# fdrmrc/fictitious_domain_AL_preconditioners

Hardware: AMD Instinct MI355X
Metric: FGMRES iterations/sec to 1e-8 residual, 3D Stokes-immersed (AL-preconditioned) (higher is better)
Workload: dtype f64

## Files before the change

### fictitious_domain_al_preconditioners_amd/_abi.py

```python
import ctypes as C

ALFD_MAX_BLOCKS = 3

OK, E_INVALID, E_HIP, E_NO_CONVERGENCE_OUTER, E_NO_CONVERGENCE_INNER, E_BREAKDOWN, E_NOT_SETUP, \
    E_COMM, E_UNSUPPORTED = range(9)
A, BT, B, CT, C_, M, MP, A2, KIMM = range(9)
NSLOTS = 9
SLOT_BY_NAME = {"A": A, "Bt": BT, "B": B, "Ct": CT, "C": C_, "M": M, "Mp": MP, "A2": A2, "K": KIMM}
INVW, MP_LUMPED_INV = 0, 1
NDIAGS = 2
AL2, AL_STOKES, AL_STOKES_DIAG, AL_ELL_IDEAL, AL_ELL_MODIFIED, RATIONAL = range(6)
CTRL_ABS, CTRL_REDUCTION, CTRL_FIXED_ITERS = range(3)
PREC_IDENTITY, PREC_JACOBI, PREC_CHEBYSHEV, PREC_MULTILEVEL = range(4)
INNER_OP_AUG, INNER_OP_A22, INNER_OP_AUG2 = range(3)
SPECTRUM_CCT = 0
ORTH_MGS, ORTH_CGS, ORTH_CGS2 = range(3)
OUTER_FGMRES, OUTER_MINRES = range(2)
FGMRES_DEALII_96, FGMRES_DEALII_95 = range(2)
W_DIAGONAL, W_MASS_INV_SQUARED, W_MASS_INV = range(3)
INNER_THROW, INNER_ACCEPT = range(2)
T_SPMV_A, T_SPMV_OTHER, T_DOT, T_VEC = range(4)
T_NCLASSES = 4
SC_PRODUCTS_A, SC_PRODUCTS_C, SC_LEVEL_A_UPLOADS, SC_TRANSFER_UPLOADS, SC_PATCH_BUILDS, SC_POWER_ITERATIONS = range(6)
SC_NCOUNTS = 6
SETUP_COUNT_NAMES = ("products_a", "products_c", "level_a_uploads", "transfer_uploads", "patch_builds",
                     "power_iterations")
UNIQUE_ID_BYTES = 128


class Control(C.Structure):
    _fields_ = [("kind", C.c_int32), ("max_steps", C.c_int32), ("tol", C.c_double), ("reduce", C.c_double)]

    def __init__(self, kind=CTRL_ABS, max_steps=100, tol=1e-10, reduce=0.0):
        super().__init__(kind, max_steps, tol, reduce)


class Config(C.Structure):
    _fields_ = [
        ("variant", C.c_int32), ("restart", C.c_int32), ("orthogonalization", C.c_int32),
        ("grad_div_in_A", C.c_int32),
        ("gamma", C.c_double), ("gamma_grad_div", C.c_double), ("gamma2", C.c_double),
        ("outer", Control), ("inner", Control), ("mp_inner", Control),
        ("inner_prec", C.c_int32), ("cheb_degree", C.c_int32), ("cheb_power_its", C.c_int32),
        ("on_inner_failure", C.c_int32),
        ("cheb_eig_ratio", C.c_double), ("cheb_safety", C.c_double),
        ("log_level", C.c_int32), ("outer_solver", C.c_int32),
        ("rho_bound", C.c_double), ("rational", Control),
        ("ml_smooth_degree", C.c_int32), ("ml_coarse_degree", C.c_int32),
        ("ml_smooth_ratio", C.c_double), ("ml_coarse_ratio", C.c_double),
        ("aug_assembled", C.c_int32), ("w_inverse", C.c_int32),
        ("mass", Control),
        ("fgmres_flavour", C.c_int32), ("ml_smooth_degree_coarse", C.c_int32),
        ("ml_patch_degree", C.c_int32), ("ml_coarse_direct", C.c_int32), ("ml_patch_ratio", C.c_double),
    ]


class Result(C.Structure):
    _fields_ = [
        ("status", C.c_int32), ("outer_iterations", C.c_int32),
        ("initial_residual", C.c_double), ("last_residual", C.c_double),
        ("inner_iterations", C.c_int64), ("mp_iterations", C.c_int64),
        ("inner_failures", C.c_int32), ("precond_applications", C.c_int32),
        ("solve_seconds", C.c_double), ("lambda_max", C.c_double),
        ("rational_iterations", C.c_int64), ("mass_iterations", C.c_int64),
    ]

    def as_dict(self):
        return {k: getattr(self, k) for k, _ in self._fields_}


class Spectrum(C.Structure):
    _fields_ = [
        ("converged", C.c_int32), ("steps", C.c_int32),
        ("initial_residual", C.c_double), ("last_residual", C.c_double),
        ("lambda_min", C.c_double), ("lambda_max", C.c_double), ("condition", C.c_double),
    ]

    def as_dict(self):
        return {k: getattr(self, k) for k, _ in self._fields_}


class MatrixInfo(C.Structure):
    _fields_ = [
        ("lanes", C.c_int32), ("windowed", C.c_int32), ("value_indexed", C.c_int32), ("batch_major", C.c_int32),
        ("nnz", C.c_int64), ("window_blocks", C.c_int64), ("window_fallback_blocks", C.c_int64),
        ("value_indexed_blocks", C.c_int64), ("value_indexed_nnz", C.c_int64),
        ("dictionary_entries", C.c_int64), ("value_wide_nnz", C.c_int64),
        ("algorithmic_bytes", C.c_double), ("streamed_bytes", C.c_double),
        ("shared_nnz", C.c_int64), ("batch_major_blocks", C.c_int64), ("batch_major_wide", C.c_int64),
        ("batch_major_interior_blocks", C.c_int64),
    ]


class BatchMajorShape(C.Structure):
    _fields_ = [
        ("batch_major", C.c_int32), ("lanes", C.c_int32),
        ("nrows", C.c_int64), ("nnz", C.c_int64), ("shared_nnz", C.c_int64),
        ("rows", C.c_int64), ("waves", C.c_int64), ("small", C.c_int64),
        ("blocks", C.c_int64), ("batches", C.c_int64), ("lds_bytes", C.c_int64), ("compute_units", C.c_int64),
    ]

    def as_dict(self):
        plain = ("batch_major", "lanes", "nrows", "nnz", "shared_nnz")
        return {(k if k in plain else "batch_major_" + k): getattr(self, k) for k, _ in self._fields_}


OPERATOR_LEVEL, OPERATOR_PATCH_SS, OPERATOR_PATCH_S = 0, 1, 2


class WindowPlanInfo(C.Structure):
    _fields_ = [
        ("windowed", C.c_int32), ("value_indexed", C.c_int32), ("row_block", C.c_int32), ("max_window", C.c_int32),
        ("blocks", C.c_int64), ("fallback_blocks", C.c_int64), ("segments", C.c_int64),
        ("value_indexed_blocks", C.c_int64), ("value_indexed_nnz", C.c_int64), ("value_wide_nnz", C.c_int64),
        ("dictionary_entries", C.c_int64), ("batches", C.c_int64), ("decode_mismatches", C.c_int64),
    ]


class StreamPlanInfo(C.Structure):
    _fields_ = [
        ("ok", C.c_int32), ("max_window", C.c_int32), ("max_rows", C.c_int32), ("max_batches", C.c_int32),
        ("blocks", C.c_int64), ("batches", C.c_int64), ("segments", C.c_int64), ("dictionary_entries", C.c_int64),
        ("stream_bytes", C.c_int64), ("decode_mismatches", C.c_int64), ("rows_covered", C.c_int64),
        ("shared_nnz", C.c_int64),
    ]


def default_config(variant=AL_STOKES) -> Config:
    c = Config()
    c.variant = variant
    c.restart = 50 if variant in (AL_ELL_IDEAL, AL_ELL_MODIFIED) else 30
    c.orthogonalization = ORTH_CGS2
    c.grad_div_in_A = 1
    c.gamma, c.gamma_grad_div, c.gamma2 = 10.0, 10.0, 1e-2
    c.outer = Control(CTRL_REDUCTION, 1000, 1e-8, 1e-12)
    c.inner = Control(CTRL_ABS, 100, 1e-2, 0.0)
    c.mp_inner = Control(CTRL_ABS, 100, 1e-6, 0.0)
    c.inner_prec = PREC_CHEBYSHEV
    c.cheb_degree = 4
    c.cheb_power_its = 20
    c.on_inner_failure = INNER_THROW
    c.cheb_eig_ratio = 30.0
    c.cheb_safety = 1.2
    c.log_level = 0
    c.outer_solver = OUTER_MINRES if variant == RATIONAL else OUTER_FGMRES
    c.rho_bound = 0.0
    c.rational = Control(CTRL_ABS, 2000, 1e-14, 0.0)
    c.ml_smooth_degree, c.ml_coarse_degree = 3, 40
    c.ml_smooth_ratio, c.ml_coarse_ratio = 4.0, 400.0
    c.w_inverse = W_DIAGONAL
    c.mass = Control(CTRL_REDUCTION, 1000, 1e-30, 1e-14)
    c.ml_patch_degree, c.ml_coarse_direct, c.ml_patch_ratio = 0, 0, 30.0
    return c


def bench_multilevel_settings(cfg: Config, geometric: bool = True) -> Config:
    cfg.inner_prec = PREC_MULTILEVEL
    cfg.inner.max_steps = 100
    cfg.ml_coarse_degree = 10
    if geometric:
        cfg.ml_smooth_degree, cfg.ml_smooth_degree_coarse, cfg.ml_smooth_ratio = 3, 5, 40.0
        cfg.ml_patch_degree, cfg.ml_patch_ratio, cfg.ml_coarse_direct = 15, 200.0, 1024
    else:
        cfg.ml_smooth_degree, cfg.ml_smooth_degree_coarse, cfg.ml_smooth_ratio = 4, 0, 256.0
        cfg.ml_patch_degree, cfg.ml_coarse_direct = 0, 0
    return cfg


BENCH_MIN_COARSE = 1024
```

### fictitious_domain_al_preconditioners_amd/csrc/alfd.hip

```cpp

#include <hip/hip_runtime.h>
#include <rccl/rccl.h>

#include <algorithm>
#include <atomic>
#include <chrono>
#include <cmath>
#include <cstdio>
#include <cstdlib>
#include <cstring>
#include <memory>
#include <climits>
#include <condition_variable>
#include <functional>
#include <limits>
#include <mutex>
#include <string>
#include <thread>
#include <unordered_set>
#include <vector>

#include "alfd/alfd.h"
#include "kernels.hpp"
#include "kernels_vs.hpp"

namespace alfd {


#define HIPC(call)                                                                          \
  do {                                                                                      \
    hipError_t e__ = (call);                                                                \
    if (e__ != hipSuccess) {                                                                \
      ctx->err = std::string(#call) + ": " + hipGetErrorString(e__) + " (" + __FILE__ + ":" + \
                 std::to_string(__LINE__) + ")";                                            \
      return ALFD_E_HIP;                                                                    \
    }                                                                                       \
  } while (0)
#define RC(call)                  \
  do {                            \
    int rc__ = (call);            \
    if (rc__ != ALFD_OK) return rc__; \
  } while (0)

static inline int64_t pad_chunk(int64_t n) { return (n + kChunk - 1) / kChunk * kChunk; }

struct DevCsr {
  bool present = false;
  int64_t nrows = 0, ncols = 0, nnz = 0;
  int64_t n_list = 0;
  bool sparse = false;
  bool rep = false;
  bool derived = false;
  int L = 64;
  int32_t n_local_cols = 0;
  int64_t *rp = nullptr;
  int32_t *col = nullptr;
  double *val = nullptr;
  int32_t *rows = nullptr;
  std::vector<int64_t> send_off, recv_off;
  std::vector<int32_t> halo_globals;
  int32_t *send_idx = nullptr;
  double *send_buf = nullptr, *halo = nullptr;
  int64_t n_halo = 0;
  std::vector<void *> owned;
  bool win = false;
  bool win_deferred = false, win_user = true;
  int tag = 0;
  int32_t win_RB = 0, win_maxW = 0;
  int64_t win_nblocks = 0, win_fallback_blocks = 0, win_nseg = 0;
  uint16_t *lcol = nullptr;
  bool vi = false;
  uint8_t *vidx = nullptr;
  int32_t *blk_dict_off = nullptr, *blk_dict_n = nullptr;
  double *dict = nullptr;
  int64_t vi_blocks = 0, vi_nnz = 0, vi_dict_total = 0, vi_wide_nnz = 0;
  uint16_t *vidw = nullptr;
  uint64_t *vib_tab = nullptr;
  int32_t *vib_cnt = nullptr;
  int32_t vib_stride = 0;
  int32_t *blk_seg_begin = nullptr, *blk_W = nullptr, *seg_col = nullptr, *seg_off = nullptr;
  struct Vs {
    bool on = false, bricks = false;
    int64_t nb = 0, nseg = 0, stream_bytes = 0, nbatch = 0, dict_total = 0, shared_nnz = 0;
    int32_t stride = 0, maxW = 0;
    int32_t L = 64, tab_u64 = 16;
    int32_t wide = 0;
    int32_t RB = 0, NW = 4;
    bool small = false;
    uint8_t *stream = nullptr;
    int64_t *sb = nullptr;
    uint64_t *tab = nullptr;
    int32_t *cnt = nullptr, *seg_begin = nullptr, *blkW = nullptr, *seg_col = nullptr,
            *seg_off = nullptr, *doff = nullptr, *dn = nullptr;
    int32_t *hdrb = nullptr, *segx = nullptr;
    int32_t seg_stride = 0;
    int64_t nb_interior = 0;
    double *dict = nullptr;
  } vs;
  double streamed_bytes(bool use_vi, bool use_vs = false) const {
    const double vec = (double)(n_list + 1) * 8.0 + (double)n_list * 8.0 + (double)(sparse ? n_list : ncols) * 8.0;
    if (vs.on && use_vs && use_vi)
      return (double)vs.stream_bytes + 8.0 * vs.tab_u64 * (double)vs.nbatch + 28.0 * (double)vs.nb +
             8.0 * (double)vs.nseg + 8.0 * (double)vs.dict_total + 8.0 * (double)nrows +
             8.0 * (double)(sparse ? n_list : ncols);
    if (!win) return (double)nnz * 12.0 + vec;
    const double meta = (double)win_nblocks * 8.0 + (double)win_nseg * 8.0;
    if (!(vi && use_vi)) return (double)nnz * 10.0 + vec + meta;
    return (double)(vi_nnz - vi_wide_nnz) * 3.0 + (double)vi_wide_nnz * 4.0 + (double)(nnz - vi_nnz) * 10.0 + vec + meta + (double)vi_dict_total * 8.0 +
           (double)win_nblocks * (8.0 + (vib_tab ? 32.0 * vib_stride + 4.0 : 0.0));
  }
  double algorithmic_bytes() const {
    return (double)nnz * 12.0 + (double)(n_list + 1) * 8.0 + (double)n_list * 8.0 +
           (double)(sparse ? n_list : ncols) * 8.0;
  }
};

struct HostCsr {
  int64_t nrows = 0, ncols = 0;
  std::vector<int64_t> rp;
  std::vector<int32_t> col;
  std::vector<double> val;
  int64_t nnz() const { return rp.empty() ? 0 : rp.back(); }
};

constexpr int kScratchSlot = ALFD_NSLOTS;

struct LevelStore {
  DevCsr A, C, Ct;
  DevCsr P, R;
  int64_t n = 0, npad = 0;
  double *dinv = nullptr, *r = nullptr, *z = nullptr, *t = nullptr, *cd = nullptr, *cres = nullptr, *ctmp = nullptr;
};

struct MlLevel {
  LevelStore loc, rep;
  double lmax = 0;
  uint8_t *tail_mask = nullptr;
  bool P_global_cols = false;
  std::vector<int64_t> offs;
  int64_t maxpiece = 0;
  double *send = nullptr, *stage = nullptr;
};

enum State { ITERATE = 0, SUCCESS = 1, FAILURE = 2 };
struct Control {
  alfd_control c;
  double initial = 0, reduced_tol = 0, last_value = 0;
  int last_step = 0;
  State check(int step, double v) {
    last_step = step;
    last_value = v;
    if (step == 0) {
      initial = v;
      reduced_tol = v * c.reduce;
    }
    if (c.kind == ALFD_CTRL_REDUCTION && v < reduced_tol) return SUCCESS;
    if (c.kind == ALFD_CTRL_FIXED_ITERS && step >= c.max_steps) return SUCCESS;
    if (v <= c.tol) return SUCCESS;
    if (step >= c.max_steps || std::isnan(v)) return FAILURE;
    return ITERATE;
  }
};

struct TimedLaunch {
  int cls;
  hipEvent_t a, b;
};

}

using namespace alfd;

struct alfd_ctx {
  int device = 0;
  hipStream_t stream = nullptr;
  hipStream_t xstream = nullptr;
  hipEvent_t ev_x = nullptr, ev_halo = nullptr;
  hipEvent_t ev_in = nullptr;
  int overlap_halo = -1;
  std::string err;
  int rank = 0, nranks = 1;
  ncclComm_t nccl = nullptr;
// ... 56 lines not shown
    void clear_input() {
      for (int l = 0; l < ALFD_MAX_LEVELS; ++l) agg[l].clear(), wgt[l].clear(), P[l] = HostCsr(), ncoarse[l] = 0;
      built_partitioned = false;
    }
  } hier[2];
  struct Patch {
    bool on = false;
    int64_t m = 0, mpad = 0;
    DevCsr Ass, As, Ats, Cs, Cts;
    int32_t *S = nullptr;
    double *dinv = nullptr, *rS = nullptr, *zS = nullptr, *uS = nullptr, *eS = nullptr, *cd = nullptr,
           *cres = nullptr, *ctmp = nullptr, *rr = nullptr;
    double lmax = 0;
    uint8_t *tail_mask = nullptr;
    bool rep = false;
    int64_t m_loc = 0, piece = 1, lam_piece = 1;
    std::vector<int64_t> soff;
    DevCsr Cts_loc, Ctg;
    double *send = nullptr, *stage = nullptr, *lam_send = nullptr, *lam_stage = nullptr, *loc = nullptr;
  } patch;
  struct StrengthGraph {
    bool have = false, on_device = false;
    int64_t n_nodes = 0, node0 = 0;
    std::vector<int64_t> gp;
    std::vector<int32_t> gc, fixed;
    std::vector<double> gw, d;
  } sg;
  int ml_rep_level = -1;
  bool dots_replicated = false;
  int64_t ml_rep_threshold = 300000;
  int ml_fuse = 2;
  int ml_tail_rows = 0;
  int ml_gpu_galerkin = 1;
  double *g_w = nullptr, *g_tlam = nullptr;
  std::vector<int64_t> ml_coff[ALFD_MAX_LEVELS];
  const int64_t *up_col_offsets = nullptr;
  bool up_local_only = false;
  DevCsr rat_mat;
  double *rt_r = nullptr, *rt_z = nullptr, *rt_p = nullptr, *rt_Ap = nullptr, *rt_x = nullptr;
  double *rt_dinv = nullptr, *rt_partial = nullptr, *rt_scb = nullptr, *rt_coef = nullptr;
  double *rt_scb_host = nullptr;
  int64_t rational_its = 0;
  int64_t wmax = 0;
  std::vector<void *> ws_allocs;
  double *w_r = nullptr, *w_z = nullptr, *w_p = nullptr, *w_Ap = nullptr;
  double *c_d = nullptr, *c_res = nullptr, *c_tmp = nullptr;
  double *t_lam = nullptr;
  double *q_tmp = nullptr, *rhs_tmp = nullptr;
  double *V = nullptr, *Z = nullptr, *xb = nullptr, *bb = nullptr, *io = nullptr;
  double *st_in = nullptr, *st_out = nullptr;
  double lambda_max = 0, lambda_min = 0;
  int64_t inner_its = 0, mp_its = 0;
  int64_t inner_its_op[3] = {0, 0, 0};
  int inner_failures = 0, precond_applications = 0;
  std::vector<double> history;
  int timing = 0;
  std::vector<TimedLaunch> timed;
  double t_ms[ALFD_T_NCLASSES] = {0, 0, 0, 0};
  int64_t t_launches[ALFD_T_NCLASSES] = {0, 0, 0, 0};
  double t_bytes[ALFD_T_NCLASSES] = {0, 0, 0, 0};
  double t_fbytes[ALFD_T_NCLASSES] = {0, 0, 0, 0};
  double setup_s[ALFD_SETUP_NPHASES] = {0, 0, 0, 0, 0, 0, 0, 0};
  bool upload_since_setup = false;
  uint64_t gen[ALFD_NSLOTS + 1] = {}, gen_setup[ALFD_NSLOTS + 1] = {};
  uint64_t dgen[ALFD_NDIAGS] = {}, dgen_setup[ALFD_NDIAGS] = {};
  alfd_config cfg_setup;
  const char *needs_full = nullptr;
  bool coupling_ready = false;
  int64_t setup_counts[ALFD_SC_NCOUNTS] = {};
  std::vector<void *> cp_allocs[2];
  std::vector<void *> allocs;
  int spmv_stream_R = 2, spmv_stream_U = 8, spmv_nt = 0, spmv_grid_mult = 8;
  int spmv_group_R = 4, spmv_group_U = 4;
  bool vi_off = false;
  int vi_rows_R = 4, vi_rows_J = 2;
  int vi_xcd = 0;
  int vi_levels = 1;
  int vi_batched = 1;
  int win_RB_vi = 96;
  int win_vi = 1;
  int win_short_scale = 2;
  int vs_enable = 1, vs_NW = 4, vs_RB = 96, vs_xcd = 0, vs_share = 1, vs_wide = 1;
  int vs_small = 1;
  int vs_cus = 0;
  int vs_force_RB = 0, vs_force_NW = 0;
  int vs_lds_base_ok = -1;
  std::vector<int64_t> rb_ptr[ALFD_NSLOTS + 1];
  std::vector<int32_t> rb_rows[ALFD_NSLOTS + 1];
  int win_short_min_blocks = 256;
  int win_min_blocks = 256;
  int win_enable = 1, win_RB = 96, win_maxW = 4096, win_gap = 8, win_xcd = 0;
  int64_t ntot() const { return off[nblocks]; }
};

struct alfd_local_group {
  int n = 0;
  std::mutex mu;
  std::condition_variable cv;
  int arrived = 0;
  long generation = 0;
  std::vector<const void *> buf;
  std::vector<const int64_t *> off;
  void barrier() {
    std::unique_lock<std::mutex> lk(mu);
    const long g = generation;
    if (++arrived == n) {
      arrived = 0;
      ++generation;
      cv.notify_all();
    } else {
      cv.wait(lk, [&] { return generation != g; });
    }
  }
};

namespace alfd {

static int comm_allgather(alfd_ctx *ctx, const void *send, void *recv, size_t bytes) {
  if (ctx->local) {
    alfd_local_group *g = ctx->local;
    HIPC(hipStreamSynchronize(ctx->stream));
    g->buf[ctx->rank] = send;
    g->barrier();
    for (int p = 0; p < g->n; ++p)
      HIPC(hipMemcpyAsync((char *)recv + (size_t)p * bytes, g->buf[p], bytes, hipMemcpyDeviceToDevice,
                          ctx->stream));
    HIPC(hipStreamSynchronize(ctx->stream));
    g->barrier();
    return ALFD_OK;
  }
  if (ctx->host_allgather) {
    ctx->host_send.resize(bytes);
    ctx->host_recv.resize(bytes * (size_t)ctx->nranks);
    HIPC(hipMemcpyAsync(ctx->host_send.data(), send, bytes, hipMemcpyDeviceToHost, ctx->stream));
    HIPC(hipStreamSynchronize(ctx->stream));
    if (ctx->host_allgather(ctx->host_user, ctx->host_send.data(), ctx->host_recv.data(), bytes) != 0)
      return ctx->err = "host all-gather callback failed", ALFD_E_COMM;
    HIPC(hipMemcpyAsync(recv, ctx->host_recv.data(), ctx->host_recv.size(), hipMemcpyHostToDevice, ctx->stream));
    HIPC(hipStreamSynchronize(ctx->stream));
    return ALFD_OK;
  }
  if (ncclAllGather(send, recv, bytes, ncclChar, ctx->nccl, ctx->stream) != ncclSuccess)
    return ctx->err = "ncclAllGather failed", ALFD_E_COMM;
  return ALFD_OK;
}

static int comm_alltoallv(alfd_ctx *ctx, const void *sendbuf, const int64_t *send_off, void *recvbuf,
                          const int64_t *recv_off, size_t es, hipStream_t st = nullptr) {
  if (!st) st = ctx->stream;
  if (ctx->local) {
    alfd_local_group *g = ctx->local;
    HIPC(hipStreamSynchronize(st));
    g->buf[ctx->rank] = sendbuf;
    g->off[ctx->rank] = send_off;
    g->barrier();
    for (int p = 0; p < g->n; ++p) {
      const int64_t nr = recv_off[p + 1] - recv_off[p];
      if (nr > 0)
        HIPC(hipMemcpyAsync((char *)recvbuf + (size_t)recv_off[p] * es,
                            (const char *)g->buf[p] + (size_t)g->off[p][ctx->rank] * es, (size_t)nr * es,
                            hipMemcpyDeviceToDevice, st));
    }
    HIPC(hipStreamSynchronize(st));
    g->barrier();
    return ALFD_OK;
  }
// ... 56 lines not shown
  for (void *q : m.owned) hipFree(q);
  m = DevCsr();
}

static void spectrum_release(alfd_ctx *ctx) {
  csr_free(ctx->spec.own_Cs);
  csr_free(ctx->spec.own_Cts);
  for (void *q : ctx->spec.owned) hipFree(q);
  ctx->spec = alfd_ctx::Spectrum();
}

static inline int grid_for_rows(int64_t nrows, int L) {
  const int64_t groups = (nrows + (kBlock / L) - 1) / (kBlock / L);
  return (int)std::max<int64_t>(1, std::min<int64_t>(groups, 256 * 8));
}

struct Timer {
  alfd_ctx *ctx;
  int cls;
  hipEvent_t a = nullptr, b = nullptr;
  bool on;
  Timer(alfd_ctx *c, int cl, double bytes, double fbytes = -1.0) : ctx(c), cls(cl) {
    on = ctx->timing >= 2 || (ctx->timing == 1 && cl == ALFD_T_SPMV_A);
    if (on) {
      hipEventCreate(&a);
      hipEventCreate(&b);
      hipEventRecord(a, ctx->stream);
      ctx->t_bytes[cls] += bytes;
      ctx->t_fbytes[cls] += fbytes < 0.0 ? bytes : fbytes;
      ctx->t_launches[cls]++;
    }
  }
  ~Timer() {
    if (on) {
      hipEventRecord(b, ctx->stream);
      ctx->timed.push_back({cls, a, b});
    }
  }
};

struct PhaseClock {
  alfd_ctx *ctx;
  int phase;
  std::chrono::steady_clock::time_point t0 = std::chrono::steady_clock::now();
  PhaseClock(alfd_ctx *c, int ph) : ctx(c), phase(ph) {}
  ~PhaseClock() {
    hipStreamSynchronize(ctx->stream);
    ctx->setup_s[phase] += std::chrono::duration<double>(std::chrono::steady_clock::now() - t0).count();
  }
};

static void flush_timers(alfd_ctx *ctx) {
  for (auto &t : ctx->timed) {
    hipEventSynchronize(t.b);
    float ms = 0;
    hipEventElapsedTime(&ms, t.a, t.b);
    ctx->t_ms[t.cls] += ms;
    hipEventDestroy(t.a);
    hipEventDestroy(t.b);
  }
  ctx->timed.clear();
}

template <int L>
static void launch_spmv_L(alfd_ctx *ctx, const DevCsr &m, const double *x, double *y, int epi, double alpha,
                          const double *d, double *y2) {
  const int grid = grid_for_rows(m.n_list, L);
  const double *xh = m.halo;
#define ALFD_SPMV(EPI, SP)                                                                          \
  hipLaunchKernelGGL((spmv_kernel<L, EPI, SP>), dim3(grid), dim3(kBlock), 0, ctx->stream, m.n_list, \
                     m.rp, m.col, m.val, m.rows, x, xh, m.n_local_cols, y, alpha, d, y2)
  if (m.sparse) {
    if (epi == 0) ALFD_SPMV(0, true);
    else if (epi == 1) ALFD_SPMV(1, true);
    else if (epi == 2) ALFD_SPMV(2, true);
    else ALFD_SPMV(3, true);
  } else {
    if (epi == 0) ALFD_SPMV(0, false);
    else if (epi == 1) ALFD_SPMV(1, false);
    else if (epi == 2) ALFD_SPMV(2, false);
    else ALFD_SPMV(3, false);
  }
#undef ALFD_SPMV
}

template <int R, int U, bool NT>
static void launch_stream(alfd_ctx *ctx, const DevCsr &m, const double *x, double *y, int epi, double alpha,
                          const double *d, double *y2) {
  const int64_t nbatches = (m.nrows + R - 1) / R;
  const int grid = (int)std::max<int64_t>(1, std::min<int64_t>((nbatches + 3) / 4, 256 * ctx->spmv_grid_mult));
#define ALFD_STREAM(EPI)                                                                              \
  hipLaunchKernelGGL((spmv_stream_kernel<R, U, EPI, NT>), dim3(grid), dim3(kBlock), 0, ctx->stream,   \
                     m.nrows, m.rp, m.col, m.val, x, m.halo, m.n_local_cols, y, alpha, d, y2, NoPair())
  if (epi == 0) ALFD_STREAM(0);
  else if (epi == 1) ALFD_STREAM(1);
  else if (epi == 2) ALFD_STREAM(2);
  else ALFD_STREAM(3);
#undef ALFD_STREAM
}

template <bool NT>
static bool launch_stream_RU(alfd_ctx *ctx, const DevCsr &m, const double *x, double *y, int epi,
                             double alpha, const double *d, double *y2) {
  const int R = ctx->spmv_stream_R, U = ctx->spmv_stream_U;
#define ALFD_RU(RR, UU) \
  if (R == RR && U == UU) return launch_stream<RR, UU, NT>(ctx, m, x, y, epi, alpha, d, y2), true
  ALFD_RU(2, 2); ALFD_RU(2, 4); ALFD_RU(4, 2); ALFD_RU(4, 4); ALFD_RU(4, 8); ALFD_RU(8, 4); ALFD_RU(8, 8);
  ALFD_RU(1, 4); ALFD_RU(2, 8); ALFD_RU(8, 2);
#undef ALFD_RU
  return false;
}

template <int R, int U>
static void launch_window(alfd_ctx *ctx, const DevCsr &m, const double *x, double *y, int epi, double alpha,
                          const double *d, double *y2) {
  const size_t lds = (size_t)(m.win_maxW + (m.vi && !ctx->vi_off ? kDictMaxEntries : 0)) * sizeof(double);
#define ALFD_WIN(EPI, TAG)                                                                              \
  hipLaunchKernelGGL((spmv_window_kernel<R, U, EPI, TAG>), dim3((unsigned)m.win_nblocks), dim3(kBlock), \
                     lds, ctx->stream, m.nrows, m.win_RB, m.rp, m.col, m.lcol, m.val, m.blk_seg_begin,   \
                     m.blk_W, m.seg_col, m.seg_off, x, m.halo, m.n_local_cols, y, alpha, d, y2, ctx->win_xcd)
  const bool vi = m.vi && !ctx->vi_off;
  if (vi && ctx->vi_batched && m.vib_tab) {
#define ALFD_VIB(EPI, TAG)                                                                                    \
  hipLaunchKernelGGL((spmv_window_vib_kernel<EPI, TAG>), dim3((unsigned)m.win_nblocks), dim3(kBlock), lds,   \
                     ctx->stream, m.nrows, m.win_RB, m.rp, m.col, m.lcol, m.val, m.blk_seg_begin, m.blk_W,    \
                     m.seg_col, m.seg_off, x, m.halo, m.n_local_cols, y, alpha, d, y2, m.vidx, m.vidw,        \
                     m.blk_dict_off, m.blk_dict_n, m.dict, m.win_maxW, m.vib_tab, m.vib_cnt, m.vib_stride,    \
                     ctx->vi_xcd)
    if (m.tag == 0) {
      if (epi == 0) ALFD_VIB(0, 0);
      else if (epi == 1) ALFD_VIB(1, 0);
      else if (epi == 2) ALFD_VIB(2, 0);
      else ALFD_VIB(3, 0);
    } else {
      if (epi == 0) ALFD_VIB(0, 1);
      else if (epi == 1) ALFD_VIB(1, 1);
      else if (epi == 2) ALFD_VIB(2, 1);
      else ALFD_VIB(3, 1);
    }
#undef ALFD_VIB
    return;
  }
  if (vi && ctx->vi_rows_R > 0) {
    const int RR = ctx->vi_rows_R, JJ = ctx->vi_rows_J;
#define ALFD_VI(RV, JV, EPI)                                                                                  \
  hipLaunchKernelGGL((spmv_window_vi_kernel<RV, JV, EPI>), dim3((unsigned)m.win_nblocks), dim3(kBlock), lds,  \
                     ctx->stream, m.nrows, m.win_RB, m.rp, m.col, m.lcol, m.val, m.blk_seg_begin, m.blk_W,     \
                     m.seg_col, m.seg_off, x, m.halo, m.n_local_cols, y, alpha, d, y2, m.vidx, m.vidw, \
                     m.blk_dict_off, m.blk_dict_n, m.dict, m.win_maxW)
#define ALFD_VI_E(RV, JV)              \
  if (RR == RV && JJ == JV) {          \
    if (epi == 0) ALFD_VI(RV, JV, 0);  \
    else if (epi == 1) ALFD_VI(RV, JV, 1); \
    else if (epi == 2) ALFD_VI(RV, JV, 2); \
    else ALFD_VI(RV, JV, 3);           \
    return;                            \
  }
    ALFD_VI_E(4, 3) ALFD_VI_E(2, 4) ALFD_VI_E(4, 4)
    if (epi == 0) ALFD_VI(4, 2, 0);
    else if (epi == 1) ALFD_VI(4, 2, 1);
    else if (epi == 2) ALFD_VI(4, 2, 2);
    else ALFD_VI(4, 2, 3);
    return;
#undef ALFD_VI_E
#undef ALFD_VI
  }
// ... 92 lines not shown
      hipMemcpyAsync(&base, probe, sizeof(uint32_t), hipMemcpyDeviceToHost, ctx->stream);
      hipStreamSynchronize(ctx->stream);
      hipFree(probe);
    }
    ctx->vs_lds_base_ok = base == 0 ? 1 : 0;
    if (!ctx->vs_lds_base_ok)
      std::fprintf(stderr, "[alfd] dynamic LDS does not start at offset 0 (%u): batch-major SpMV formats disabled\n", base);
  }
  return ctx->vs_lds_base_ok != 0;
}

static bool launch_vs(alfd_ctx *ctx, const DevCsr &m, const double *x, double *y, int epi, double alpha,
                      const double *d, double *y2, int64_t first_block = 0, int64_t n_blocks = -1) {
  const DevCsr::Vs &v = m.vs;
  if (!vs_lds_base_ok(ctx)) return false;
  if (v.L == 32) return launch_vss<32>(ctx, m, x, y, epi, alpha, d, y2), true;
  if (v.L == 16) return launch_vss<16>(ctx, m, x, y, epi, alpha, d, y2), true;
  if (v.L == 8) return launch_vss<8>(ctx, m, x, y, epi, alpha, d, y2), true;
  const int NW = v.NW;
  const size_t lds = (size_t)(v.wide ? VsFmt<1>::kWinOff : VsFmt<0>::kWinOff) + (size_t)v.maxW * sizeof(double);
  if (n_blocks < 0) n_blocks = v.nb - first_block;
  if (n_blocks <= 0) return true;
  const unsigned grid = (unsigned)n_blocks;
  const int32_t base = (int32_t)first_block;
#define ALFD_VS_ARGS \
  v.stream, v.tab, v.stride, v.hdrb, v.segx, v.seg_stride, v.dict, x, m.halo, m.n_local_cols, y, alpha, d, y2, ctx->vs_xcd, base, NoPair()
#define ALFD_VS(EPI, NWV)                                                                                        \
  do {                                                                                                           \
    if (v.wide)                                     \
      hipLaunchKernelGGL((spmv_vs_kernel<EPI, 0, 4, 1>), dim3(grid), dim3(256), lds, ctx->stream,     \
                         ALFD_VS_ARGS);                                                                          \
    else if (m.tag == 0)                                                                                         \
      hipLaunchKernelGGL((spmv_vs_kernel<EPI, 0, NWV>), dim3(grid), dim3(64 * NWV), lds, ctx->stream, \
                         ALFD_VS_ARGS);                                                                          \
    else   \
      hipLaunchKernelGGL((spmv_vs_kernel<EPI, 1, (NWV > 4 ? 4 : NWV)>), dim3(grid), dim3(64 * (NWV > 4 ? 4 : NWV)), lds, \
                         ctx->stream, ALFD_VS_ARGS);                                                             \
  } while (0)
#define ALFD_VS_E(NWV)                  \
  do {                                  \
    if (epi == 0) ALFD_VS(0, NWV);      \
    else if (epi == 1) ALFD_VS(1, NWV); \
    else if (epi == 2) ALFD_VS(2, NWV); \
    else ALFD_VS(3, NWV);               \
  } while (0)
  if (NW == 8) ALFD_VS_E(8);
  else if (NW == 2) ALFD_VS_E(2);
  else if (NW == 1) ALFD_VS_E(1);
  else ALFD_VS_E(4);
#undef ALFD_VS_E
#undef ALFD_VS
#undef ALFD_VS_ARGS
  return true;
}

static int halo_exchange(alfd_ctx *ctx, DevCsr &m, const double *x, hipStream_t st = nullptr);
static int spmv_launch_local(alfd_ctx *ctx, DevCsr &m, const double *x, double *y, int epi, double alpha, const double *d,
                             double *y2);

static int spmv_m(alfd_ctx *ctx, DevCsr &m, int cls, const double *x, double *y, int epi, double alpha = 0.0,
                  const double *d = nullptr, double *y2 = nullptr) {
  if (!m.present) return ctx->err = "matrix not set", ALFD_E_NOT_SETUP;
  const bool exchange = ctx->nranks > 1 && !m.rep && (ctx->local || ctx->host_alltoallv || m.n_halo > 0 || m.send_off.back() > 0);
  const bool overlap = exchange && (ctx->overlap_halo > 0 || (ctx->overlap_halo < 0 && (ctx->local || ctx->host_alltoallv))) && ctx->xstream && m.vs.on && m.vs.L == 64 && ctx->vs_enable && !ctx->vi_off &&
                       m.vs.nb_interior > 0 && !m.sparse && m.n_list > 0;
  if (overlap) {
    Timer tm(ctx, cls, m.algorithmic_bytes(), m.streamed_bytes(true, true));
    HIPC(hipEventRecord(ctx->ev_x, ctx->stream));
    if (!launch_vs(ctx, m, x, y, epi, alpha, d, y2, 0, m.vs.nb_interior)) return ctx->err = "batch-major launch failed", ALFD_E_HIP;
    HIPC(hipStreamWaitEvent(ctx->xstream, ctx->ev_x, 0));
    RC(halo_exchange(ctx, m, x, ctx->xstream));
    HIPC(hipEventRecord(ctx->ev_halo, ctx->xstream));
    HIPC(hipStreamWaitEvent(ctx->stream, ctx->ev_halo, 0));
    launch_vs(ctx, m, x, y, epi, alpha, d, y2, m.vs.nb_interior, m.vs.nb - m.vs.nb_interior);
    HIPC(hipGetLastError());
    return ALFD_OK;
  }
  if (exchange) RC(halo_exchange(ctx, m, x));
  if (m.sparse && epi != 1) {
    HIPC(hipMemsetAsync(y, 0, m.nrows * sizeof(double), ctx->stream));
    if (epi == 3) HIPC(hipMemsetAsync(y2, 0, m.nrows * sizeof(double), ctx->stream));
  }
  if (m.n_list == 0) return ALFD_OK;
  Timer tm(ctx, cls, m.algorithmic_bytes(), m.streamed_bytes(!ctx->vi_off, ctx->vs_enable != 0 && !ctx->vi_off));
  return spmv_launch_local(ctx, m, x, y, epi, alpha, d, y2);
}

static int spmv_launch_local(alfd_ctx *ctx, DevCsr &m, const double *x, double *y, int epi, double alpha, const double *d,
                             double *y2) {
  if (m.vs.on && ctx->vs_enable && !ctx->vi_off && launch_vs(ctx, m, x, y, epi, alpha, d, y2)) {
    HIPC(hipGetLastError());
    return ALFD_OK;
  }
  if (m.win && launch_window_RU(ctx, m, x, y, epi, alpha, d, y2)) {
    HIPC(hipGetLastError());
    return ALFD_OK;
  }
  if (m.L == 64 && !m.sparse && ctx->spmv_stream_R > 0) {
    const bool ok = ctx->spmv_nt ? launch_stream_RU<true>(ctx, m, x, y, epi, alpha, d, y2)
                                 : launch_stream_RU<false>(ctx, m, x, y, epi, alpha, d, y2);
    if (ok) {
      HIPC(hipGetLastError());
      return ALFD_OK;
    }
  }
  switch (m.L) {
    case 4: launch_spmv_L<4>(ctx, m, x, y, epi, alpha, d, y2); break;
    case 8: launch_spmv_L<8>(ctx, m, x, y, epi, alpha, d, y2); break;
    case 16: launch_spmv_L<16>(ctx, m, x, y, epi, alpha, d, y2); break;
    case 32: launch_spmv_L<32>(ctx, m, x, y, epi, alpha, d, y2); break;
    default: launch_spmv_L<64>(ctx, m, x, y, epi, alpha, d, y2); break;
  }
  HIPC(hipGetLastError());
  return ALFD_OK;
}

static int pick_short_row_format(alfd_ctx *ctx, DevCsr &m) {
  if (!m.vs.on || m.vs.L == 64 || m.nnz < 20000000 || ctx->vi_off || !ctx->vs_enable || m.sparse) return ALFD_OK;
  double *x = nullptr, *y = nullptr;
  const int64_t nx = std::max<int64_t>(ctx->nranks > 1 && !m.rep ? m.n_local_cols : m.ncols, 1);
  HIPC(hipMalloc((void **)&x, nx * sizeof(double)));
  HIPC(hipMalloc((void **)&y, std::max<int64_t>(m.nrows, 1) * sizeof(double)));
  HIPC(hipMemsetAsync(x, 0, nx * sizeof(double), ctx->stream));
  hipEvent_t e0, e1;
  HIPC(hipEventCreate(&e0));
  HIPC(hipEventCreate(&e1));
  float t[2] = {0.f, 0.f};
  bool ok = true;
  for (int f = 0; f < 2 && ok; ++f) {
    for (int it = 0; it < 6 && ok; ++it) {
      if (it == 1) hipEventRecord(e0, ctx->stream);
      m.vs.on = f == 0;
      ok = spmv_launch_local(ctx, m, x, y, 0, 0.0, nullptr, nullptr) == ALFD_OK;
    }
    m.vs.on = true;
    hipEventRecord(e1, ctx->stream);
    hipEventSynchronize(e1);
    hipEventElapsedTime(&t[f], e0, e1);
  }
  hipEventDestroy(e0);
  hipEventDestroy(e1);
  hipFree(x);
  hipFree(y);
  HIPC(hipGetLastError());
  if (ok && t[1] < 0.9f * t[0]) {
    m.vs.on = false;
    if (ctx->cfg.log_level > 0 || std::getenv("ALFD_LOG_UPLOAD"))
      std::fprintf(stderr, "[alfd] short-row operator (%lld rows, %lld nnz): without the batch-major form %.3f ms, with it %.3f ms per launch "
                   "-> batch-major form dropped\n", (long long)m.nrows, (long long)m.nnz, t[1] / 5.0, t[0] / 5.0);
  }
  return ALFD_OK;
}

static int spmv(alfd_ctx *ctx, int slot, const double *x, double *y, int epi, double alpha = 0.0,
                const double *d = nullptr, double *y2 = nullptr) {
  DevCsr &m = ctx->mat[slot];
  if (!m.present) return ctx->err = "matrix slot " + std::to_string(slot) + " not set", ALFD_E_NOT_SETUP;
  return spmv_m(ctx, m, slot == ALFD_A ? ALFD_T_SPMV_A : ALFD_T_SPMV_OTHER, x, y, epi, alpha, d, y2);
}

static bool tail_form(const DevCsr &m) { return m.present && !m.vs.on && !m.win; }


static int pair_form_A(alfd_ctx *ctx, const DevCsr &A) {
  if (!A.present || A.sparse || A.n_list == 0) return 0;
  if (A.vs.on && ctx->vs_enable && !ctx->vi_off)
    return A.vs.L == 64 && !A.vs.wide && A.vs.NW <= 4 && A.vs.nb > 0 && vs_lds_base_ok(ctx) ? 1 : 0;
  if (A.win) return 0;
  return A.L == 64 && ctx->spmv_stream_R == 2 && ctx->spmv_stream_U == 8 && !ctx->spmv_nt ? 2 : 0;
}

static inline bool gd_nested(const alfd_ctx *ctx);
static int pair_forms(alfd_ctx *ctx, const DevCsr &A, const DevCsr &C) {
  const bool ok = ctx->nranks == 1 && ctx->cfg.w_inverse == ALFD_W_DIAGONAL && !ctx->cfg.aug_assembled && !gd_nested(ctx) &&
                  tail_form(C) && !C.sparse && C.nrows > 0 && (C.L == 16 || C.L == 32 || C.L == 64) && A.ncols == C.ncols;
  return ok ? pair_form_A(ctx, A) : 0;
}
static int pair_ok(alfd_ctx *ctx, const DevCsr &A, const DevCsr &C) {
  const bool fine = &A == &ctx->mat[ALFD_A] || &A == &ctx->mat[ALFD_A2];
  return ctx->ml_fuse >= (fine ? 3 : 2) ? pair_forms(ctx, A, C) : 0;
}

static int launch_pair(alfd_ctx *ctx, int form, const DevCsr &A, int clsA, const DevCsr &C, const double *w,
                       const double *x, double *y, double *t) {
  const bool vi = !ctx->vi_off, vs = ctx->vs_enable != 0 && !ctx->vi_off;
  Timer tm(ctx, clsA, A.algorithmic_bytes() + C.algorithmic_bytes(), A.streamed_bytes(vi, vs) + C.streamed_bytes(vi, vs));
  PairC pc;
  pc.nrows = C.n_list, pc.rp = C.rp, pc.col = C.col, pc.val = C.val, pc.x_halo = C.halo, pc.d = w, pc.t = t;
  pc.n_local = C.n_local_cols, pc.L = C.L;
  pc.nC = (uint32_t)grid_for_rows(C.n_list, C.L);
  if (form == 1) {
    const DevCsr::Vs &v = A.vs;
    const size_t lds = (size_t)VsFmt<0>::kWinOff + (size_t)v.maxW * sizeof(double);
    pc.nA = (uint32_t)v.nb;
    const int64_t rpb = 64 * v.NW / C.L;
    pc.nC = (uint32_t)std::max<int64_t>(1, std::min<int64_t>((C.n_list + rpb - 1) / rpb, 256 * 8));
#define ALFD_VS_PAIR(TAG, NWV)                                                                                             \
  hipLaunchKernelGGL((spmv_vs_kernel<0, TAG, NWV, 0, true>), dim3(pc.nA + pc.nC), dim3(64 * NWV), lds, ctx->stream,       \
                     v.stream, v.tab, v.stride, v.hdrb, v.segx, v.seg_stride, v.dict, x, A.halo, A.n_local_cols, y, 0.0,  \
                     (const double *)nullptr, (double *)nullptr, ctx->vs_xcd, 0, pc)
#define ALFD_VS_PAIR_T(TAG)              \
  do {                                   \
    if (v.NW == 1) ALFD_VS_PAIR(TAG, 1); \
    else if (v.NW == 2) ALFD_VS_PAIR(TAG, 2); \
    else ALFD_VS_PAIR(TAG, 4);           \
  } while (0)
    if (A.tag == 0) ALFD_VS_PAIR_T(0);
    else ALFD_VS_PAIR_T(1);
#undef ALFD_VS_PAIR_T
#undef ALFD_VS_PAIR
  } else {
    const int64_t nbatches = (A.nrows + 1) / 2;
    pc.nA = (uint32_t)std::max<int64_t>(1, std::min<int64_t>((nbatches + 3) / 4, 256 * ctx->spmv_grid_mult));
    hipLaunchKernelGGL((spmv_stream_kernel<2, 8, 0, false, true>), dim3(pc.nA + pc.nC), dim3(kBlock), 0, ctx->stream,
                       A.nrows, A.rp, A.col, A.val, x, A.halo, A.n_local_cols, y, 0.0, (const double *)nullptr,
                       (double *)nullptr, pc);
  }
  HIPC(hipGetLastError());
  return ALFD_OK;
}

static int spmv_AC(alfd_ctx *ctx, DevCsr &A, int clsA, DevCsr &C, const double *w, const double *x, double *y, double *t) {
  if (const int form = pair_ok(ctx, A, C)) return launch_pair(ctx, form, A, clsA, C, w, x, y, t);
  RC(spmv_m(ctx, A, clsA, x, y, 0));
  return spmv_m(ctx, C, ALFD_T_SPMV_OTHER, x, t, 2, 0.0, w);
}

static int finish_dots(alfd_ctx *ctx, int64_t nb, int count, int out, int fin) {
  if (ctx->nranks == 1 || ctx->dots_replicated) {
    hipLaunchKernelGGL(dot_final_kernel, dim3(count), dim3(kBlock), 0, ctx->stream, ctx->partial, nb,
                       ctx->pstride, ctx->sc, out, fin);
    HIPC(hipGetLastError());
// ... 2074 lines not shown
  for (int64_t b = 0; b < pl.nb; ++b) {
    const int32_t s0 = pl.seg_begin[b], ns = pl.seg_begin[b + 1] - s0;
    int32_t *h = &hdrb[(size_t)b * 8];
    h[0] = pl.cnt[b];
    h[1] = pl.blkW[b];
    h[2] = ns;
    h[3] = pl.dn[b];
    h[4] = pl.doff[b];
    h[5] = (int32_t)(uint32_t)((uint64_t)pl.sb[b] & 0xffffffffull);
    h[6] = (int32_t)((uint64_t)pl.sb[b] >> 32);
    for (int32_t q = 0; q < ns; ++q) {
      segx[((size_t)b * S + q) * 2] = pl.seg_col[s0 + q];
      segx[((size_t)b * S + q) * 2 + 1] = pl.seg_off[s0 + q];
    }
  }
  pl.tab.resize(pl.tab.size() + (size_t)16 * kVsBatchRows, 0);
  RC(upload_vec(ctx, m, &v.stream, pl.stream));
  RC(upload_vec(ctx, m, &v.tab, pl.tab));
  RC(upload_vec(ctx, m, &v.hdrb, hdrb));
  RC(upload_vec(ctx, m, &v.segx, segx));
  RC(upload_vec(ctx, m, &v.dict, pl.dict));
  HIPC(hipStreamSynchronize(ctx->stream));
  v.seg_stride = S;
  v.nb_interior = pl.nb_interior;
  v.nb = pl.nb;
  v.nseg = (int64_t)pl.seg_col.size();
  v.stream_bytes = (int64_t)pl.stream.size() - 4096;
  v.nbatch = pl.nbatch;
  v.shared_nnz = pl.shared_nnz;
  v.dict_total = (int64_t)pl.dict.size();
  v.stride = pl.stride;
  v.maxW = pl.maxW;
  v.wide = pl.wide;
  v.bricks = hint;
  v.on = true;
  if (ctx->cfg.log_level > 0)
    std::fprintf(stderr,
                 "[alfd] batch-major format%s: %lld blocks (%s), %lld batches, window <= %d slots, %.2f B/nnz, %.1f %% of the "
                 "entries in template-shared batches\n", pl.wide ? " (10-bit codes)" : "",
                 (long long)pl.nb, hint ? "caller's row blocks" : "runs of the numbering", (long long)pl.nbatch, pl.maxW,
                 (double)v.stream_bytes / (double)std::max<int64_t>(m.nnz, 1),
                 100.0 * (double)pl.shared_nnz / (double)std::max<int64_t>(m.nnz, 1));
  return ALFD_OK;
}

static int build_vss(alfd_ctx *ctx, DevCsr &m, const int64_t *rp, const int32_t *col, const double *val) {
  VsPlan pl;
  const int RB = std::min(kVssMaxRows, std::max(64, ctx->win_RB * std::max(1, ctx->win_short_scale) * 64 / m.L));
  plan_vss(m.nrows, m.L, rp, col, val, RB, ctx->win_maxW, ctx->win_gap, pl);
  if (!pl.ok || pl.shared_nnz * 2 < m.nnz) return ALFD_OK;
  DevCsr::Vs &v = m.vs;
  RC(upload_vec(ctx, m, &v.stream, pl.stream));
  RC(upload_vec(ctx, m, &v.sb, pl.sb));
  RC(upload_vec(ctx, m, &v.tab, pl.tab));
  RC(upload_vec(ctx, m, &v.cnt, pl.cnt));
  RC(upload_vec(ctx, m, &v.seg_begin, pl.seg_begin));
  RC(upload_vec(ctx, m, &v.blkW, pl.blkW));
  RC(upload_vec(ctx, m, &v.seg_col, pl.seg_col));
  RC(upload_vec(ctx, m, &v.seg_off, pl.seg_off));
  RC(upload_vec(ctx, m, &v.doff, pl.doff));
  RC(upload_vec(ctx, m, &v.dn, pl.dn));
  RC(upload_vec(ctx, m, &v.dict, pl.dict));
  HIPC(hipStreamSynchronize(ctx->stream));
  v.nb = pl.nb;
  v.nseg = (int64_t)pl.seg_col.size();
  v.stream_bytes = (int64_t)pl.stream.size() - 4096;
  v.nbatch = pl.nbatch;
  v.shared_nnz = pl.shared_nnz;
  v.dict_total = (int64_t)pl.dict.size();
  v.stride = pl.stride;
  v.maxW = pl.maxW;
  v.L = m.L;
  v.tab_u64 = 1 + 4 * (64 / m.L);
  v.bricks = false;
  v.on = true;
  if (ctx->cfg.log_level > 0)
    std::fprintf(stderr, "[alfd] batch-major format (L = %d): %lld blocks, %lld batches, window <= %d slots, %.2f B/nnz, "
                 "%.1f %% of the entries in shared batches\n", m.L, (long long)pl.nb, (long long)pl.nbatch, pl.maxW,
                 (double)(v.stream_bytes + 8.0 * v.tab_u64 * v.nbatch) / (double)std::max<int64_t>(m.nnz, 1),
                 100.0 * (double)pl.shared_nnz / (double)std::max<int64_t>(m.nnz, 1));
  return ALFD_OK;
}

static int upload_matrix(alfd_ctx *ctx, int slot, int64_t nrows, int64_t ncols, const int64_t *rp,
                         const int32_t *col, const double *val) {
  DevCsr &m = ctx->mat[slot];
  csr_free(m);
  const auto t_up0 = std::chrono::steady_clock::now();
  m.nrows = nrows;
  m.ncols = ncols;
  m.nnz = rp[nrows];
  int64_t nonempty = 0;
  for (int64_t r = 0; r < nrows; ++r) nonempty += rp[r + 1] > rp[r];
  m.sparse = nonempty * 2 < nrows;
  if (ctx->nranks > 1) {
    int64_t mine[2] = {m.nnz, nonempty};
    std::vector<int64_t> all(2 * (size_t)ctx->nranks);
    int64_t *d_m = nullptr, *d_a = nullptr;
    HIPC(hipMalloc((void **)&d_m, 2 * sizeof(int64_t)));
    HIPC(hipMalloc((void **)&d_a, 2 * sizeof(int64_t) * ctx->nranks));
    HIPC(hipMemcpyAsync(d_m, mine, sizeof(mine), hipMemcpyHostToDevice, ctx->stream));
    RC(comm_allgather(ctx, d_m, d_a, sizeof(mine)));
    HIPC(hipMemcpyAsync(all.data(), d_a, all.size() * 8, hipMemcpyDeviceToHost, ctx->stream));
    HIPC(hipStreamSynchronize(ctx->stream));
    hipFree(d_m);
    hipFree(d_a);
    int64_t gn = 0, ge = 0;
    for (int p = 0; p < ctx->nranks; ++p) gn += all[2 * p], ge += all[2 * p + 1];
    DevCsr tmp;
    tmp.nnz = gn;
    choose_lanes(tmp, ge);
    m.L = tmp.L;
  } else {
    choose_lanes(m, nonempty);
  }
  const int32_t *col_up = col;
  std::vector<int32_t> remap;
  m.n_local_cols = (int32_t)ncols;
  if (ctx->nranks > 1 && ctx->up_local_only) {
    m.send_off.assign(ctx->nranks + 1, 0);
    m.recv_off.assign(ctx->nranks + 1, 0);
  } else if (ctx->nranks > 1) {
    if (ctx->part.empty()) return ctx->err = "alfd_set_partition must precede alfd_set_matrix", ALFD_E_INVALID;
    int rb, cb;
    slot_blocks(ctx, slot, &rb, &cb);
    const int64_t *po = ctx->up_col_offsets ? ctx->up_col_offsets : ctx->part[cb].data();
    const int64_t c0 = po[ctx->rank], c1 = po[ctx->rank + 1];
    m.n_local_cols = (int32_t)(c1 - c0);
    std::vector<int32_t> hal;
    remap.resize(m.nnz);
    m.recv_off.assign(ctx->nranks + 1, 0);
    host_halo_plan(m.nnz, col, po, ctx->nranks, ctx->rank, remap.data(), hal, m.recv_off.data());
    m.n_halo = (int64_t)hal.size();
    m.halo_globals = hal;
    col_up = remap.data();
    std::vector<int32_t> cnt_local(ctx->nranks), cnt_all((size_t)ctx->nranks * ctx->nranks);
    for (int p = 0; p < ctx->nranks; ++p) cnt_local[p] = (int32_t)(m.recv_off[p + 1] - m.recv_off[p]);
    int32_t *d_cl = nullptr, *d_ca = nullptr;
    HIPC(hipMalloc((void **)&d_cl, sizeof(int32_t) * ctx->nranks));
    HIPC(hipMalloc((void **)&d_ca, sizeof(int32_t) * ctx->nranks * ctx->nranks));
    HIPC(hipMemcpyAsync(d_cl, cnt_local.data(), ctx->nranks * 4, hipMemcpyHostToDevice, ctx->stream));
    RC(comm_allgather(ctx, d_cl, d_ca, (size_t)ctx->nranks * 4));
    HIPC(hipMemcpyAsync(cnt_all.data(), d_ca, cnt_all.size() * 4, hipMemcpyDeviceToHost, ctx->stream));
    HIPC(hipStreamSynchronize(ctx->stream));
    m.send_off.assign(ctx->nranks + 1, 0);
    for (int p = 0; p < ctx->nranks; ++p)
      m.send_off[p + 1] = m.send_off[p] + cnt_all[(size_t)p * ctx->nranks + ctx->rank];
    const int64_t nsend = m.send_off.back();
    int32_t *d_req = nullptr, *d_want = nullptr;
    HIPC(hipMalloc((void **)&d_req, sizeof(int32_t) * std::max<int64_t>(m.n_halo, 1)));
    HIPC(hipMalloc((void **)&d_want, sizeof(int32_t) * std::max<int64_t>(nsend, 1)));
    HIPC(hipMemcpyAsync(d_req, hal.data(), m.n_halo * 4, hipMemcpyHostToDevice, ctx->stream));
    RC(comm_alltoallv(ctx, d_req, m.recv_off.data(), d_want, m.send_off.data(), sizeof(int32_t)));
    std::vector<int32_t> want(nsend);
    HIPC(hipMemcpyAsync(want.data(), d_want, nsend * 4, hipMemcpyDeviceToHost, ctx->stream));
    HIPC(hipStreamSynchronize(ctx->stream));
    hipFree(d_cl);
    hipFree(d_ca);
    hipFree(d_req);
    hipFree(d_want);
    for (auto &g : want) g = (int32_t)(g - c0);
    RC(csr_alloc(ctx, m, &m.send_idx, nsend));
    HIPC(hipMemcpyAsync(m.send_idx, want.data(), nsend * 4, hipMemcpyHostToDevice, ctx->stream));
    RC(csr_alloc(ctx, m, &m.send_buf, nsend));
    RC(csr_alloc(ctx, m, &m.halo, m.n_halo));
    HIPC(hipStreamSynchronize(ctx->stream));
  }
  RC(csr_alloc(ctx, m, &m.col, m.nnz));
  RC(csr_alloc(ctx, m, &m.val, m.nnz));
  struct CopyJob {
    std::thread th;
    hipError_t rc = hipSuccess;
    ~CopyJob() { if (th.joinable()) th.join(); }
  } copy_job;
  if (m.nnz > 50000000) {
    const int dev = ctx->device;
    int32_t *dcol = m.col;
    double *dval = m.val;
    const int64_t nn = m.nnz;
    copy_job.th = std::thread([&copy_job, dev, dcol, dval, col_up, val, nn] {
      hipStream_t st = nullptr;
      hipError_t e = hipSetDevice(dev);
      if (e == hipSuccess) e = hipStreamCreateWithFlags(&st, hipStreamNonBlocking);
      if (e == hipSuccess) e = hipMemcpyAsync(dcol, col_up, nn * sizeof(int32_t), hipMemcpyHostToDevice, st);
      if (e == hipSuccess) e = hipMemcpyAsync(dval, val, nn * sizeof(double), hipMemcpyHostToDevice, st);
      if (e == hipSuccess) e = hipStreamSynchronize(st);
      if (st) hipStreamDestroy(st);
      copy_job.rc = e;
    });
  } else {
    HIPC(hipMemcpyAsync(m.col, col_up, m.nnz * sizeof(int32_t), hipMemcpyHostToDevice, ctx->stream));
    HIPC(hipMemcpyAsync(m.val, val, m.nnz * sizeof(double), hipMemcpyHostToDevice, ctx->stream));
  }
  if (m.sparse) {
    std::vector<int32_t> rows;
    std::vector<int64_t> crp(1, 0);
    for (int64_t r = 0; r < nrows; ++r)
      if (rp[r + 1] > rp[r]) {
        rows.push_back((int32_t)r);
        crp.push_back(rp[r + 1]);
      }
    for (size_t i = 0; i < rows.size(); ++i) crp[i] = rp[rows[i]];
    crp[rows.size()] = m.nnz;
    m.n_list = (int64_t)rows.size();
    RC(csr_alloc(ctx, m, &m.rows, m.n_list));
    RC(csr_alloc(ctx, m, &m.rp, m.n_list + 1));
    HIPC(hipMemcpyAsync(m.rows, rows.data(), m.n_list * sizeof(int32_t), hipMemcpyHostToDevice, ctx->stream));
    HIPC(hipMemcpyAsync(m.rp, crp.data(), (m.n_list + 1) * sizeof(int64_t), hipMemcpyHostToDevice,
                        ctx->stream));
    HIPC(hipStreamSynchronize(ctx->stream));
  } else {
    m.n_list = nrows;
    RC(csr_alloc(ctx, m, &m.rp, nrows + 1));
    HIPC(hipMemcpyAsync(m.rp, rp, (nrows + 1) * sizeof(int64_t), hipMemcpyHostToDevice, ctx->stream));
  }
  HIPC(hipStreamSynchronize(ctx->stream));
  const bool win_long = m.L == 64 && m.nrows >= (int64_t)ctx->win_RB * ctx->win_min_blocks;
  const bool win_short = ctx->win_short_scale > 0 && m.L >= 8 && m.L < 64 &&
                         m.nrows >= (int64_t)std::min(512, ctx->win_RB * ctx->win_short_scale * 64 / m.L) * ctx->win_short_min_blocks;
  const bool windows = ctx->win_enable && (win_long || win_short) && !m.sparse && m.nnz > 0;
  const auto t_plan0 = std::chrono::steady_clock::now();
  if (windows && ctx->vs_enable && ctx->win_vi && m.L == 64 && (slot != kScratchSlot || ctx->vi_levels))
    RC(build_vs(ctx, m, slot, rp, col_up, val));
  const auto t_plan1 = std::chrono::steady_clock::now();
  m.win_deferred = windows && m.vs.on && m.L == 64;
  m.win_user = slot != kScratchSlot;
  if (windows && !m.win_deferred) RC(build_window(ctx, m, rp, col_up, val, slot != kScratchSlot, m.vs.on));
  if ((ctx->cfg.log_level > 0 || std::getenv("ALFD_LOG_UPLOAD")) && m.nnz > 50000000)
    std::fprintf(stderr, "[alfd] upload of a %lld-nnz matrix: CSR copy %.2f s, batch-major plan + copy %.2f s, window plan + copy %.2f s\n",
                 (long long)m.nnz, std::chrono::duration<double>(t_plan0 - t_up0).count(),
                 std::chrono::duration<double>(t_plan1 - t_plan0).count(),
                 std::chrono::duration<double>(std::chrono::steady_clock::now() - t_plan1).count());
  if (ctx->vs_enable && windows && !m.sparse && (m.L == 32 || m.L == 16 || m.L == 8)) RC(build_vss(ctx, m, rp, col_up, val));
  if (copy_job.th.joinable()) {
    copy_job.th.join();
    if (copy_job.rc != hipSuccess) return ctx->err = hipGetErrorString(copy_job.rc), ALFD_E_HIP;
  }
  m.present = true;
  RC(pick_short_row_format(ctx, m));
  return ALFD_OK;
}

static int upload_transpose(alfd_ctx *ctx, int slot, int64_t nrows, int64_t ncols, const int64_t *rp,
                            const int32_t *col, const double *val) {
  const int64_t nnz = rp[nrows];
  std::vector<int64_t> trp(ncols + 1, 0);
  std::vector<int32_t> tcol(nnz);
  std::vector<double> tval(nnz);
  for (int64_t k = 0; k < nnz; ++k) trp[col[k] + 1]++;
  for (int64_t r = 0; r < ncols; ++r) trp[r + 1] += trp[r];
  std::vector<int64_t> cur(trp.begin(), trp.end() - 1);
  for (int64_t r = 0; r < nrows; ++r)
    for (int64_t k = rp[r]; k < rp[r + 1]; ++k) {
      const int64_t p = cur[col[k]]++;
      tcol[p] = (int32_t)r;
      tval[p] = val[k];
    }
  return upload_matrix(ctx, slot, ncols, nrows, trp.data(), tcol.data(), tval.data());
}

static int nblocks_of(int variant) { return variant == ALFD_AL2 || variant == ALFD_RATIONAL ? 2 : 3; }

static int ws_alloc_zero(alfd_ctx *ctx, double **p, int64_t count, std::vector<void *> *list = nullptr) {
  void *q = nullptr;
  HIPC(hipMalloc(&q, std::max<int64_t>(count, 1) * sizeof(double)));
  (list ? *list : ctx->ws_allocs).push_back(q);
  *p = static_cast<double *>(q);
  HIPC(hipMemsetAsync(q, 0, std::max<int64_t>(count, 1) * sizeof(double), ctx->stream));
  return ALFD_OK;
}
static int cp_alloc_zero(alfd_ctx *ctx, int h, double **p, int64_t count) {
  return ws_alloc_zero(ctx, p, count, &ctx->cp_allocs[h]);
}
static void cp_release(alfd_ctx *ctx, int h) {
  for (void *p : ctx->cp_allocs[h]) hipFree(p);
  ctx->cp_allocs[h].clear();
}

static int diag_plus_m(alfd_ctx *ctx, const DevCsr *A, DevCsr &R, const double *w, double g, int64_t n, double *dinv,
                       bool invert);
static int diag_plus_m(alfd_ctx *ctx, const DevCsr &A, DevCsr &R, double g, int64_t n, double *dinv) {
  return diag_plus_m(ctx, &A, R, ctx->diag[ALFD_INVW], g, n, dinv, true);
}
static int diag_plus(alfd_ctx *ctx, int slot_diag, int slot_rows, double g, int64_t n, double *dinv) {
  return diag_plus_m(ctx, ctx->mat[slot_diag], ctx->mat[slot_rows], g, n, dinv);
}
static int diag_plus_m(alfd_ctx *ctx, const DevCsr *A, DevCsr &R, const double *w, double g, int64_t n, double *dinv,
                       bool invert) {
  if (A && pad_chunk(n) > ctx->diag_cap) {
    RC(ws_alloc_zero(ctx, &ctx->dA, pad_chunk(n)));
    RC(ws_alloc_zero(ctx, &ctx->s_aug, pad_chunk(n)));
    ctx->diag_cap = pad_chunk(n);
  }
  if (A) HIPC(hipMemsetAsync(ctx->dA, 0, pad_chunk(n) * sizeof(double), ctx->stream));
  HIPC(hipMemsetAsync(ctx->s_aug, 0, pad_chunk(n) * sizeof(double), ctx->stream));
  if (A) {
    const int grid = grid_for_rows(A->nrows, A->L);
#define ALFD_DIAG(LL)                                                                                      \
  hipLaunchKernelGGL((extract_diag_kernel<LL>), dim3(grid), dim3(kBlock), 0, ctx->stream, A->nrows, A->rp, \
                     A->col, A->val, ctx->dA)
    switch (A->L) {
      case 4: ALFD_DIAG(4); break;
      case 8: ALFD_DIAG(8); break;
      case 16: ALFD_DIAG(16); break;
      case 32: ALFD_DIAG(32); break;
      default: ALFD_DIAG(64); break;
    }
#undef ALFD_DIAG
  }
  if (ctx->nranks > 1 && (ctx->local || ctx->host_alltoallv || R.n_halo > 0 || R.send_off.back() > 0))
    RC(halo_exchange(ctx, R, w));
  if (R.n_list > 0)
    hipLaunchKernelGGL(aug_diag_rows_kernel, dim3((unsigned)((R.n_list + 255) / 256)), dim3(256), 0,
                       ctx->stream, R.n_list, R.rp, R.col, R.val, R.sparse ? R.rows : nullptr,
                       w, R.halo, R.n_local_cols, ctx->s_aug);
  hipLaunchKernelGGL(aug_diag_finish_kernel, dim3((unsigned)std::max<int64_t>(1, (n + 255) / 256)), dim3(256), 0, ctx->stream, n,
                     g, ctx->dA, ctx->s_aug, dinv, invert ? 1 : 0);
  HIPC(hipGetLastError());
  return ALFD_OK;
}

// ... 3197 lines not shown
  ctx->rational_its = 0;
  ctx->mass_its = 0;
}
static void fill_result(alfd_ctx *ctx, alfd_result *res, int status) {
  res->status = status;
  res->inner_iterations = ctx->inner_its;
  res->mp_iterations = ctx->mp_its;
  res->inner_failures = ctx->inner_failures;
  res->precond_applications = ctx->precond_applications;
  res->lambda_max = ctx->lambda_max;
  res->rational_iterations = ctx->rational_its;
  res->mass_iterations = ctx->mass_its;
}

}

static void hierarchy_input_changed(alfd_ctx *ctx) {
  ctx->is_setup = false;
  ctx->needs_full = "a prolongator, aggregates or a row-block hint was set";
}

#define CHECK_CTX()                       \
  if (!ctx) return ALFD_E_INVALID;        \
  if (hipSetDevice(ctx->device) != hipSuccess) return ctx->err = "hipSetDevice failed", ALFD_E_HIP
#define CHECK_SETUP() \
  if (!ctx->is_setup) return ctx->err = "alfd_setup not called", ALFD_E_NOT_SETUP

extern "C" {

int alfd_abi_version(void) { return ALFD_ABI_VERSION; }

const char *alfd_strerror(int s) {
  switch (s) {
    case ALFD_OK: return "ok";
    case ALFD_E_INVALID: return "invalid argument";
    case ALFD_E_HIP: return "HIP runtime error";
    case ALFD_E_NO_CONVERGENCE_OUTER: return "FGMRES: no convergence (SolverControl::NoConvergence)";
    case ALFD_E_NO_CONVERGENCE_INNER: return "inner CG: no convergence (SolverControl::NoConvergence)";
    case ALFD_E_BREAKDOWN: return "breakdown (NaN residual)";
    case ALFD_E_NOT_SETUP: return "context not set up";
    case ALFD_E_COMM: return "RCCL error";
    case ALFD_E_UNSUPPORTED: return "not implemented";
    default: return "unknown status";
  }
}

const char *alfd_last_error(alfd_ctx_t ctx) { return ctx ? ctx->err.c_str() : "null context"; }

int alfd_create(alfd_ctx_t *out, int device_id) {
  if (!out) return ALFD_E_INVALID;
  *out = nullptr;
  int ndev = 0;
  if (hipGetDeviceCount(&ndev) != hipSuccess || ndev <= 0 || device_id < 0 || device_id >= ndev)
    return ALFD_E_HIP;
  if (hipSetDevice(device_id) != hipSuccess) return ALFD_E_HIP;
  alfd_ctx *ctx = new alfd_ctx;
  ctx->device = device_id;
  if (hipStreamCreateWithFlags(&ctx->xstream, hipStreamNonBlocking) != hipSuccess ||
      hipEventCreateWithFlags(&ctx->ev_x, hipEventDisableTiming) != hipSuccess ||
      hipEventCreateWithFlags(&ctx->ev_halo, hipEventDisableTiming) != hipSuccess)
    ctx->xstream = nullptr;
  if (const char *e = std::getenv("ALFD_SPMV_OVERLAP_HALO")) ctx->overlap_halo = std::atoi(e);
  if (hipStreamCreateWithFlags(&ctx->stream, hipStreamNonBlocking) != hipSuccess) {
    delete ctx;
    return ALFD_E_HIP;
  }
  alfd_default_config(&ctx->cfg, ALFD_AL_STOKES);
  if (const char *e = std::getenv("ALFD_SPMV_STREAM_R")) ctx->spmv_stream_R = std::atoi(e);
  if (const char *e = std::getenv("ALFD_SPMV_STREAM_U")) ctx->spmv_stream_U = std::atoi(e);
  if (const char *e = std::getenv("ALFD_SPMV_NT")) ctx->spmv_nt = std::atoi(e);
  if (const char *e = std::getenv("ALFD_SPMV_GRID")) ctx->spmv_grid_mult = std::max(1, std::atoi(e));
  if (const char *e = std::getenv("ALFD_SPMV_WINDOW")) ctx->win_enable = std::atoi(e);
  if (const char *e = std::getenv("ALFD_SPMV_WINDOW_RB")) ctx->win_RB = std::max(4, std::atoi(e));
  if (const char *e = std::getenv("ALFD_SPMV_WINDOW_MIN_BLOCKS")) ctx->win_min_blocks = std::max(1, std::atoi(e));
  if (const char *e = std::getenv("ALFD_SPMV_WINDOW_SHORT_MIN_BLOCKS")) ctx->win_short_min_blocks = std::max(1, std::atoi(e));
  if (const char *e = std::getenv("ALFD_SPMV_WINDOW_MAXW")) ctx->win_maxW = std::min(16384, std::max(256, std::atoi(e)));
  if (const char *e = std::getenv("ALFD_ML_REPLICATE")) ctx->ml_rep_threshold = std::atoll(e);
  if (const char *e = std::getenv("ALFD_ML_GPU_GALERKIN")) ctx->ml_gpu_galerkin = std::atoi(e);
  if (const char *e = std::getenv("ALFD_ML_FUSE")) ctx->ml_fuse = std::max(0, std::min(3, std::atoi(e)));
  if (const char *e = std::getenv("ALFD_SPMV_VI_LEVELS")) ctx->vi_levels = std::atoi(e);
  if (const char *e = std::getenv("ALFD_SPMV_BATCH_MAJOR")) ctx->vs_enable = std::atoi(e);
  if (const char *e = std::getenv("ALFD_SPMV_BATCH_MAJOR_ROWS")) ctx->vs_RB = std::max(4, std::min(kVsMaxRows, std::atoi(e)));
  if (const char *e = std::getenv("ALFD_SPMV_SMALL_SHAPES")) ctx->vs_small = std::atoi(e) != 0;
  {
    hipDeviceProp_t prop;
    if (hipGetDeviceProperties(&prop, device_id) == hipSuccess) ctx->vs_cus = prop.multiProcessorCount;
  }
  if (const char *e = std::getenv("ALFD_SPMV_VI_XCD")) ctx->vi_xcd = std::atoi(e);
  if (const char *e = std::getenv("ALFD_SPMV_VI_BATCHED")) ctx->vi_batched = std::atoi(e);
  if (const char *e = std::getenv("ALFD_SPMV_WINDOW_RB_VI")) ctx->win_RB_vi = std::atoi(e);
  if (const char *e = std::getenv("ALFD_SPMV_VI_R")) ctx->vi_rows_R = std::atoi(e);
  if (const char *e = std::getenv("ALFD_SPMV_VI_J")) ctx->vi_rows_J = std::atoi(e);
  if (const char *e = std::getenv("ALFD_SPMV_VALUE_INDEX")) ctx->win_vi = std::atoi(e);
  if (const char *e = std::getenv("ALFD_SPMV_GROUP_R")) ctx->spmv_group_R = std::atoi(e);
  if (const char *e = std::getenv("ALFD_SPMV_GROUP_U")) ctx->spmv_group_U = std::atoi(e);
  if (const char *e = std::getenv("ALFD_SPMV_WINDOW_SHORT")) ctx->win_short_scale = std::max(0, std::atoi(e));
  if (const char *e = std::getenv("ALFD_SPMV_WINDOW_GAP")) ctx->win_gap = std::max(1, std::atoi(e));
  if (const char *e = std::getenv("ALFD_SPMV_WINDOW_XCD")) ctx->win_xcd = std::atoi(e);
  *out = ctx;
  return ALFD_OK;
}

int alfd_destroy(alfd_ctx_t ctx) {
  if (!ctx) return ALFD_E_INVALID;
  hipSetDevice(ctx->device);
  hipStreamSynchronize(ctx->stream);
  flush_timers(ctx);
  free_levels(ctx);
  spectrum_release(ctx);
  csr_free(ctx->rat_mat);
  for (DevCsr &m : ctx->mat) csr_free(m);
  for (void *p : ctx->ws_allocs) hipFree(p);
  for (void *p : ctx->allocs) hipFree(p);
  if (ctx->sc_host) hipHostFree(ctx->sc_host);
  if (ctx->n_sc_host) hipHostFree(ctx->n_sc_host);
  if (ctx->rt_scb_host) hipHostFree(ctx->rt_scb_host);
  if (ctx->nccl) ncclCommDestroy(ctx->nccl);
  if (ctx->xstream) hipStreamDestroy(ctx->xstream);
  if (ctx->ev_x) hipEventDestroy(ctx->ev_x);
  if (ctx->ev_halo) hipEventDestroy(ctx->ev_halo);
  if (ctx->ev_in) hipEventDestroy(ctx->ev_in);
  hipStreamDestroy(ctx->stream);
  delete ctx;
  return ALFD_OK;
}

int alfd_comm_unique_id(void *id_out, size_t bytes) {
  static_assert(sizeof(ncclUniqueId) <= ALFD_UNIQUE_ID_BYTES, "unique id size");
  if (!id_out || bytes < sizeof(ncclUniqueId)) return ALFD_E_INVALID;
  ncclUniqueId id;
  if (ncclGetUniqueId(&id) != ncclSuccess) return ALFD_E_COMM;
  std::memset(id_out, 0, bytes);
  std::memcpy(id_out, &id, sizeof(id));
  return ALFD_OK;
}

int alfd_comm_init(alfd_ctx_t ctx, int rank, int nranks, const void *id, size_t bytes) {
  CHECK_CTX();
  if (nranks < 1 || rank < 0 || rank >= nranks) return ALFD_E_INVALID;
  ctx->rank = rank;
  ctx->nranks = nranks;
  if (nranks == 1) return ALFD_OK;
  if (!id || bytes < sizeof(ncclUniqueId)) return ALFD_E_INVALID;
  ncclUniqueId uid;
  std::memcpy(&uid, id, sizeof(uid));
  if (ncclCommInitRank(&ctx->nccl, nranks, uid, rank) != ncclSuccess)
    return ctx->err = "ncclCommInitRank failed", ALFD_E_COMM;
  if (rank == 0) {
    int v = 0;
    if (ncclGetVersion(&v) == ncclSuccess) std::fprintf(stderr, "[alfd] RCCL version %d, %d ranks\n", v, nranks);
  }
  return ALFD_OK;
}

int alfd_local_group_create(int nranks, alfd_local_group **out) {
  if (!out || nranks < 1) return ALFD_E_INVALID;
  alfd_local_group *g = new alfd_local_group;
  g->n = nranks;
  g->buf.assign(nranks, nullptr);
  g->off.assign(nranks, nullptr);
  *out = g;
  return ALFD_OK;
}

int alfd_local_group_destroy(alfd_local_group *g) {
  if (!g) return ALFD_E_INVALID;
// ... 1451 lines not shown
    const int64_t k0 = rp[r0], k1 = rp[r1];
    const int32_t W = pl.blkW[b];
    if (W >= 0) {
      wcol.assign(W, -1);
      for (int32_t sg = pl.seg_begin[b]; sg < pl.seg_begin[b + 1]; ++sg) {
        const int32_t end = (sg + 1 < pl.seg_begin[b + 1]) ? pl.seg_off[sg + 1] : W;
        for (int32_t o = pl.seg_off[sg]; o < end; ++o) wcol[o] = pl.seg_col[sg] + (o - pl.seg_off[sg]);
      }
      for (int64_t k = k0; k < k1; ++k) bad += pl.lcol[k] >= W || wcol[pl.lcol[k]] != col[k];
    }
    if (pl.vi && W >= 0 && pl.blk_dn[b] >= 0) {
      const bool wide = (pl.blk_dn[b] & kDictWide) != 0;
      const int32_t nd = pl.blk_dn[b] & 0xffff;
      for (int64_t k = k0; k < k1; ++k) {
        const int32_t code = wide ? (int32_t)pl.vidw[k] : (int32_t)pl.vidx[k];
        if (code >= nd || std::memcmp(&pl.dict[pl.doff[b] + code], &val[k], 8) != 0) ++bad;
      }
    }
    if (pl.stride > 0) {
      seen.assign(r1 - r0, 0);
      batches += pl.cnt[b];
      for (int32_t q = 0; q < pl.cnt[b]; ++q) {
        const uint64_t *dsc = &pl.tab[((size_t)b * pl.stride + q) * 4];
        const int cls = (int)(dsc[0] >> 56);
        for (int i = 0; i < 4; ++i) {
          const int id = (int)((dsc[i] >> 48) & 0xff);
          const int64_t ks = (int64_t)(dsc[i] & 0xffffffffull), len = (int64_t)((dsc[i] >> 32) & 0xffff);
          if ((int)(dsc[i] >> 56) != cls) ++bad;
          if (id == 0xff) {
            bad += ks != (int64_t)(dsc[0] & 0xffffffffull) || i == 0;
            continue;
          }
          if (id >= r1 - r0) {
            ++bad;
            continue;
          }
          ++seen[id];
          const int64_t rl = rp[r0 + id + 1] - rp[r0 + id];
          const int64_t want_cls = std::min<int64_t>((rl + 63) / 64, kVibMaxClass + 1);
          bad += ks != rp[r0 + id] - k0 || len != rl || cls != want_cls;
        }
      }
      for (int v : seen) bad += v != 1;
    }
  }
  out->batches = batches;
  out->decode_mismatches = bad;
  return ALFD_OK;
}

static void shape_of(const alfd_ctx *ctx, const DevCsr &m, alfd_batch_major_shape *out) {
  std::memset(out, 0, sizeof(*out));
  const bool on = m.vs.on && ctx->vs_enable, lng = on && m.vs.L == 64;
  out->batch_major = on ? (m.vs.bricks ? 2 : 1) : 0;
  out->lanes = m.L;
  out->nrows = m.nrows;
  out->nnz = m.nnz;
  out->shared_nnz = m.vs.on ? m.vs.shared_nnz : 0;
  out->rows = lng ? m.vs.RB : 0;
  out->waves = lng ? (m.tag == 1 && m.vs.NW > 4 ? 4 : m.vs.NW) : 0;
  out->small = lng && m.vs.small ? 1 : 0;
  out->blocks = m.vs.on ? m.vs.nb : 0;
  out->batches = m.vs.on ? m.vs.nbatch : 0;
  out->compute_units = ctx->vs_cus;
  out->lds_bytes = lng ? (int64_t)(m.vs.wide ? VsFmt<1>::kWinOff : VsFmt<0>::kWinOff) + 8 * (int64_t)m.vs.maxW : 0;
}

int alfd_get_matrix_shape(alfd_ctx_t ctx, int slot, alfd_batch_major_shape *out) {
  CHECK_CTX();
  if (slot < 0 || slot >= ALFD_NSLOTS || !ctx->mat[slot].present || !out) return ALFD_E_INVALID;
  shape_of(ctx, ctx->mat[slot], out);
  return ALFD_OK;
}

static DevCsr *own_operator(alfd_ctx *ctx, int op, int level) {
  DevCsr *m = nullptr;
  if (op == ALFD_OPERATOR_LEVEL) {
    std::vector<MlLevel> &ml = ctx->hier[0].ml;
    if (level < 1 || level >= (int)ml.size()) return nullptr;
    m = ml[level].rep.A.present ? &ml[level].rep.A : &ml[level].loc.A;
  } else if (op == ALFD_OPERATOR_PATCH_SS || op == ALFD_OPERATOR_PATCH_S) {
    if (!ctx->patch.on) return nullptr;
    m = op == ALFD_OPERATOR_PATCH_SS ? &ctx->patch.Ass : &ctx->patch.As;
  }
  return m && m->present ? m : nullptr;
}

int alfd_get_operator_shape(alfd_ctx_t ctx, int op, int level, alfd_batch_major_shape *out) {
  CHECK_CTX();
  CHECK_SETUP();
  const DevCsr *m = own_operator(ctx, op, level);
  if (!m || !out) return ALFD_E_INVALID;
  shape_of(ctx, *m, out);
  return ALFD_OK;
}

int alfd_host_small_shape(int64_t nrows, int64_t blocks, int64_t batches, int32_t rows, int32_t waves, int32_t compute_units,
                          int32_t *rows_out, int32_t *waves_out) {
  if (!rows_out || !waves_out || rows < 4 || rows > kVsMaxRows || waves < 1 || compute_units < 1) return ALFD_E_INVALID;
  int r = rows, w = waves;
  vs_small_shape(nrows, blocks, batches, rows, waves, compute_units, &r, &w);
  *rows_out = r;
  *waves_out = w;
  return ALFD_OK;
}

int alfd_bench_operator(alfd_ctx_t ctx, int op, int level, int32_t rows, int32_t waves, int32_t reps, double *us_per_launch,
                        alfd_batch_major_shape *info) {
  CHECK_CTX();
  CHECK_SETUP();
  if (ctx->nranks > 1) return ALFD_E_UNSUPPORTED;
  DevCsr *own = own_operator(ctx, op, level);
  if (!own || reps < 1) return ALFD_E_INVALID;
  if (rows != 0 && (rows < 4 || rows > kVsMaxRows || (waves != 1 && waves != 2 && waves != 4))) return ALFD_E_INVALID;
  if (!own->vs.on || own->vs.L != 64 || own->sparse) return ctx->err = "not a long-row batch-major operator", ALFD_E_UNSUPPORTED;
  DevCsr tmp;
  struct Guard {
    DevCsr &t;
    ~Guard() { csr_free(t); }
  } guard{tmp};
  const DevCsr *m = own;
  if (rows != 0) {
    HostCsr h;
    RC(download_csr(ctx, *own, h));
    tmp.nrows = tmp.n_list = own->nrows, tmp.ncols = own->ncols, tmp.nnz = own->nnz;
    tmp.L = 64, tmp.tag = own->tag, tmp.n_local_cols = own->n_local_cols, tmp.rep = own->rep;
    ctx->vs_force_RB = rows, ctx->vs_force_NW = waves;
    const int rc = build_vs(ctx, tmp, kScratchSlot, h.rp.data(), h.col.data(), h.val.data());
    ctx->vs_force_RB = ctx->vs_force_NW = 0;
    RC(rc);
    if (!tmp.vs.on) return ctx->err = "the operator does not take the batch-major form at this shape", ALFD_E_UNSUPPORTED;
    tmp.present = true;
    m = &tmp;
  }
  double *dx = nullptr, *dy = nullptr;
  HIPC(hipMalloc((void **)&dx, std::max<int64_t>(m->ncols, 1) * sizeof(double)));
  HIPC(hipMalloc((void **)&dy, std::max<int64_t>(m->nrows, 1) * sizeof(double)));
  hipLaunchKernelGGL(hash_vector_kernel, dim3((unsigned)std::max<int64_t>(1, (m->ncols + 255) / 256)), dim3(256), 0, ctx->stream,
                     m->ncols, (int64_t)0, dx);
  hipEvent_t a = nullptr, b = nullptr;
  float ms = 0;
  bool ok = hipEventCreate(&a) == hipSuccess && hipEventCreate(&b) == hipSuccess;
  ok = ok && launch_vs(ctx, *m, dx, dy, 0, 0.0, nullptr, nullptr);
  ok = ok && hipEventRecord(a, ctx->stream) == hipSuccess;
  for (int i = 0; ok && i < reps; ++i) ok = launch_vs(ctx, *m, dx, dy, 0, 0.0, nullptr, nullptr);
  ok = ok && hipEventRecord(b, ctx->stream) == hipSuccess && hipEventSynchronize(b) == hipSuccess &&
       hipEventElapsedTime(&ms, a, b) == hipSuccess;
  hipStreamSynchronize(ctx->stream);
  if (a) hipEventDestroy(a);
  if (b) hipEventDestroy(b);
  hipFree(dx);
  hipFree(dy);
  HIPC(hipGetLastError());
  if (!ok) return ctx->err = "alfd_bench_operator: launch or timing failed", ALFD_E_HIP;
  if (us_per_launch) *us_per_launch = 1000.0 * (double)ms / reps;
  if (info) shape_of(ctx, *m, info);
  return ALFD_OK;
}

int alfd_get_matrix_info(alfd_ctx_t ctx, int slot, alfd_matrix_info *out) {
  CHECK_CTX();
  if (slot < 0 || slot >= ALFD_NSLOTS || !ctx->mat[slot].present || !out) return ALFD_E_INVALID;
  const DevCsr &m = ctx->mat[slot];
  std::memset(out, 0, sizeof(*out));
  out->lanes = m.L;
  out->windowed = (m.win || m.win_deferred) ? 1 : 0;
  out->value_indexed = (m.vi || (m.vs.on && ctx->vs_enable)) ? 1 : 0;
  out->batch_major = (m.vs.on && ctx->vs_enable) ? (m.vs.bricks ? 2 : 1) : 0;
  out->nnz = m.nnz;
  out->window_blocks = m.win_nblocks;
  out->window_fallback_blocks = m.win_fallback_blocks;
  out->value_indexed_blocks = m.vi_blocks;
  out->value_indexed_nnz = m.vs.on && ctx->vs_enable ? m.nnz : m.vi_nnz;
  out->dictionary_entries = m.vi_dict_total;
  out->value_wide_nnz = m.vi_wide_nnz;
  out->algorithmic_bytes = m.algorithmic_bytes();
  out->streamed_bytes = m.streamed_bytes(true, ctx->vs_enable != 0);
  out->shared_nnz = m.vs.on ? m.vs.shared_nnz : 0;
  out->batch_major_blocks = m.vs.on ? m.vs.nb : 0;
  out->batch_major_wide = m.vs.on ? m.vs.wide : 0;
  out->batch_major_interior_blocks = (m.vs.on && m.vs.L == 64 && ctx->nranks > 1 && !m.rep) ? m.vs.nb_interior : 0;
  return ALFD_OK;
}

namespace {
struct Rcb {
  int dim;
  const double *xyz;
  int64_t max_rows;
  double weight[3];
  std::vector<int32_t> idx;
  std::vector<std::vector<int64_t>> leaves;
  void split(int64_t a, int64_t e, std::vector<int64_t> &out) {
    if (e - a <= max_rows) {
      if (e > a) out.push_back(e - a);
      return;
    }
    double lo[3] = {1e300, 1e300, 1e300}, hi[3] = {-1e300, -1e300, -1e300};
    for (int64_t i = a; i < e; ++i)
      for (int d = 0; d < dim; ++d) {
        const double c = xyz[(int64_t)idx[i] * dim + d];
        lo[d] = std::min(lo[d], c);
        hi[d] = std::max(hi[d], c);
      }
    int ax = 0;
    for (int d = 1; d < dim; ++d)
      if ((hi[d] - lo[d]) * weight[d] > (hi[ax] - lo[ax]) * weight[ax]) ax = d;
    const int64_t mid = cut(a, e, ax);
    split(a, mid, out);
    split(mid, e, out);
  }
  int64_t cut(int64_t a, int64_t e, int ax) {
    const int64_t mid = a + (e - a) / 2;
    auto less = [&](int32_t p, int32_t q) {
      const double cp = xyz[(int64_t)p * dim + ax], cq = xyz[(int64_t)q * dim + ax];
      return cp < cq || (cp == cq && p < q);
    };
    std::nth_element(idx.begin() + a, idx.begin() + mid, idx.begin() + e, less);
    const double cm = xyz[(int64_t)idx[mid] * dim + ax];
    auto lo = std::partition(idx.begin() + a, idx.begin() + mid, [&](int32_t p) { return xyz[(int64_t)p * dim + ax] < cm; });
    auto hi = std::partition(idx.begin() + mid, idx.begin() + e, [&](int32_t p) { return xyz[(int64_t)p * dim + ax] <= cm; });
    const int64_t l = lo - idx.begin(), h = hi - idx.begin();
    int64_t pos = (mid - l <= h - mid) ? l : h;
    if (pos == a) pos = h;
    if (pos == e) pos = l;
    if (pos == a || pos == e) pos = mid;
    return pos;
  }
};
}

int alfd_host_row_blocks_from_points(int64_t nrows, int32_t dim, const double *points, int32_t max_rows,
                                     int64_t *n_blocks_out, int64_t *block_ptr_out, int32_t *rows_out) {
  if (nrows < 0 || dim < 1 || dim > 3 || !points || max_rows < 1 || max_rows > kVsMaxRows || !n_blocks_out ||
      !block_ptr_out || !rows_out || nrows > 2147483000LL)
    return ALFD_E_INVALID;
  Rcb r;
  r.dim = dim;
  r.xyz = points;
// ... 252 lines not shown
    i = j;
  }
  for (int64_t i = 0; i < nrows; ++i) rows_out[i] = key[i].second;
  *n_blocks_out = nb;
  return ALFD_OK;
}

int alfd_host_permute_csr(int64_t nrows, const int64_t *rp, const int32_t *col, const double *val,
                          const int64_t *row_new_to_old, const int64_t *col_old_to_new, int64_t *orp, int32_t *ocol,
                          double *oval) {
  if (nrows < 0 || !rp || !orp || (rp[nrows] > 0 && (!col || !val || !ocol || !oval))) return ALFD_E_INVALID;
  orp[0] = 0;
  for (int64_t r = 0; r < nrows; ++r) {
    const int64_t src = row_new_to_old ? row_new_to_old[r] : r;
    if (src < 0 || src >= nrows) return ALFD_E_INVALID;
    orp[r + 1] = orp[r] + (rp[src + 1] - rp[src]);
  }
  if (orp[nrows] != rp[nrows]) return ALFD_E_INVALID;
  const int T = (int)std::max<int64_t>(1, std::min<int64_t>(std::min(16u, std::max(1u, std::thread::hardware_concurrency())),
                                                           (nrows + 8191) / 8192));
  std::vector<std::thread> th;
  for (int t = 0; t < T; ++t)
    th.emplace_back([&, t]() {
      std::vector<std::pair<int32_t, double>> row;
      for (int64_t r = nrows * t / T; r < nrows * (t + 1) / T; ++r) {
        const int64_t src = row_new_to_old ? row_new_to_old[r] : r;
        const int64_t k0 = rp[src], len = rp[src + 1] - k0, o0 = orp[r];
        if (!col_old_to_new) {
          for (int64_t k = 0; k < len; ++k) ocol[o0 + k] = col[k0 + k], oval[o0 + k] = val[k0 + k];
          continue;
        }
        row.resize(len);
        for (int64_t k = 0; k < len; ++k) row[k] = {(int32_t)col_old_to_new[col[k0 + k]], val[k0 + k]};
        std::sort(row.begin(), row.end(), [](const auto &x, const auto &y) { return x.first < y.first; });
        for (int64_t k = 0; k < len; ++k) ocol[o0 + k] = row[k].first, oval[o0 + k] = row[k].second;
      }
    });
  for (auto &x : th) x.join();
  return ALFD_OK;
}

int alfd_get_device_memory(alfd_ctx_t ctx, int64_t *free_bytes, int64_t *total_bytes) {
  CHECK_CTX();
  size_t f = 0, t = 0;
  HIPC(hipMemGetInfo(&f, &t));
  if (free_bytes) *free_bytes = (int64_t)f;
  if (total_bytes) *total_bytes = (int64_t)t;
  return ALFD_OK;
}

int alfd_set_tunable(alfd_ctx_t ctx, const char *name, int value) {
  if (!ctx || !name) return ALFD_E_INVALID;
  if (std::strcmp(name, "value_index") == 0) {
    ctx->vi_off = value == 0;
    if (value == 0) RC(ensure_window_plans(ctx));
    return ALFD_OK;
  }
  if (std::strcmp(name, "batch_major") == 0) {
    ctx->vs_enable = value != 0;
    if (value == 0) RC(ensure_window_plans(ctx));
    return ALFD_OK;
  }
  if (std::strcmp(name, "batch_major_share") == 0) {
    ctx->vs_share = value != 0;
    return ALFD_OK;
  }
  if (std::strcmp(name, "batch_major_wide") == 0) {
    ctx->vs_wide = value != 0;
    return ALFD_OK;
  }
  if (std::strcmp(name, "batch_major_waves") == 0) {
    if (value != 1 && value != 2 && value != 4 && value != 8) return ctx->err = "batch_major_waves: 1, 2, 4 or 8", ALFD_E_INVALID;
    ctx->vs_NW = value;
    for (int sl = 0; sl < ALFD_NSLOTS; ++sl) {
      DevCsr::Vs &v = ctx->mat[sl].vs;
      if (v.on && v.L == 64 && !v.small && !v.wide) v.NW = value;
    }
    return ALFD_OK;
  }
  if (std::strcmp(name, "batch_major_small") == 0) {
    ctx->vs_small = value != 0;
    return ALFD_OK;
  }
  if (std::strcmp(name, "batch_major_rows") == 0) {
    if (value < 4 || value > kVsMaxRows) return ctx->err = "batch_major_rows: 4..250", ALFD_E_INVALID;
    ctx->vs_RB = value;
    return ALFD_OK;
  }
  if (std::strcmp(name, "batch_major_xcd") == 0) {
    ctx->vs_xcd = value != 0;
    return ALFD_OK;
  }
  if (std::strcmp(name, "ml_fuse") == 0) {
    ctx->ml_fuse = std::max(0, std::min(3, value));
    return ALFD_OK;
  }
  if (std::strcmp(name, "ml_gpu_galerkin") == 0) {
    if (value != 0 && value != 1) return ctx->err = "ml_gpu_galerkin: 0 or 1", ALFD_E_INVALID;
    ctx->ml_gpu_galerkin = value;
    return ALFD_OK;
  }
  if (std::strcmp(name, "ml_tail_rows") == 0) {
    if (value < 0) return ctx->err = "ml_tail_rows: >= 0", ALFD_E_INVALID;
    ctx->ml_tail_rows = value;
    return ALFD_OK;
  }
  if (std::strcmp(name, "nested_mp_group") == 0) {
    if (value < 1 || value > 1000) return ctx->err = "nested_mp_group: 1..1000", ALFD_E_INVALID;
    ctx->nmp_group = value;
    return ALFD_OK;
  }
  if (std::strcmp(name, "nested_mp_host_stepped") == 0) {
    ctx->nmp_host_stepped = value != 0;
    return ALFD_OK;
  }
  if (std::strcmp(name, "spectrum_group") == 0) {
    if (value < 1 || value > 1000) return ctx->err = "spectrum_group: 1..1000", ALFD_E_INVALID;
    ctx->spec_group = value;
    return ALFD_OK;
  }
  if (std::strcmp(name, "spectrum_host_stepped") == 0) {
    ctx->spec_host_stepped = value != 0;
    return ALFD_OK;
  }
  return ctx->err = std::string("unknown tunable ") + name, ALFD_E_INVALID;
}

int alfd_host_tridiagonal_extremes(int32_t k, const double *alpha, const double *beta, double *lambda_min,
                                   double *lambda_max) {
  return host_tridiagonal_extremes(k, alpha, beta, lambda_min, lambda_max);
}

int alfd_estimate_spectrum(alfd_ctx_t ctx, int op, const alfd_control *ctrl, alfd_spectrum *out) {
  CHECK_CTX();
  CHECK_SETUP();
  if (!out) return ALFD_E_INVALID;
  if (op != ALFD_SPECTRUM_CCT) return ctx->err = "alfd_estimate_spectrum: unknown operator", ALFD_E_INVALID;
  if (ctx->nranks > 1) return ctx->err = "alfd_estimate_spectrum: single rank only", ALFD_E_UNSUPPORTED;
  const int64_t nl = ctx->n[ctx->nblocks - 1];
  alfd_control c;
  if (ctrl) {
    c = *ctrl;
  } else {
    c.kind = ALFD_CTRL_ABS;
    c.max_steps = (int32_t)std::min<int64_t>(nl, INT32_MAX);
    c.tol = 1e-12;
    c.reduce = 0.0;
  }
  if (c.kind < ALFD_CTRL_ABS || c.kind > ALFD_CTRL_FIXED_ITERS || c.max_steps < 1)
    return ctx->err = "alfd_estimate_spectrum: bad control (max_steps >= 1)", ALFD_E_INVALID;
  if (nl < 1) return ctx->err = "alfd_estimate_spectrum: no multipliers", ALFD_E_INVALID;
  return estimate_spectrum(ctx, c, out);
}

int alfd_get_cg_coefficients(alfd_ctx_t ctx, double *alpha, double *beta, int32_t capacity, int32_t *count) {
  if (!ctx) return ALFD_E_INVALID;
  if (!ctx->spec.have) return ctx->err = "no spectrum estimate yet", ALFD_E_NOT_SETUP;
  const int32_t k = (int32_t)ctx->spec.alpha.size();
  if (count) *count = k;
  for (int32_t i = 0; i < capacity && i < k; ++i) {
    if (alpha) alpha[i] = ctx->spec.alpha[i];
    if (beta && i + 1 < k) beta[i] = ctx->spec.beta[i];
  }
  return ALFD_OK;
}

// ... 53 lines not shown
```

### fictitious_domain_al_preconditioners_amd/csrc/kernels.hpp

```cpp
#pragma once
#include <hip/hip_runtime.h>
#include <stdint.h>
#include <type_traits>

namespace alfd {

constexpr int kBlock = 256;
constexpr int64_t kChunk = 4096;
constexpr int kMaxBasis = 64;

__device__ __forceinline__ double dpp_xor_mov(double v, int which) {
  int lo = __double2loint(v), hi = __double2hiint(v), rl, rh;
  if (which == 8) {
    rl = __builtin_amdgcn_update_dpp(0, lo, 0x128, 0xf, 0xf, true);
    rh = __builtin_amdgcn_update_dpp(0, hi, 0x128, 0xf, 0xf, true);
  } else if (which == 4) {
    rl = __builtin_amdgcn_update_dpp(0, lo, 0x104, 0xf, 0x5, false);
    rl = __builtin_amdgcn_update_dpp(rl, lo, 0x114, 0xf, 0xa, false);
    rh = __builtin_amdgcn_update_dpp(0, hi, 0x104, 0xf, 0x5, false);
    rh = __builtin_amdgcn_update_dpp(rh, hi, 0x114, 0xf, 0xa, false);
  } else if (which == 2) {
    rl = __builtin_amdgcn_update_dpp(0, lo, 0x4E, 0xf, 0xf, true);
    rh = __builtin_amdgcn_update_dpp(0, hi, 0x4E, 0xf, 0xf, true);
  } else {
// ... 93 lines not shown
    p[j] = a[2 * j] + a[2 * j + 1];
  }
#pragma unroll
  for (int j = 0; j < 4; ++j) {
    swap16(p[2 * j], p[2 * j + 1]);
    u[j] = p[2 * j] + p[2 * j + 1];
    u[j] = u[j] + dpp_xor_mov(u[j], 8);
  }
  const bool h = (lane & 8) != 0;
  double x0 = h ? u[1] : u[0], x1 = h ? u[3] : u[2];
  x0 = x0 + dpp_shl<4>(x0);
  x1 = x1 + dpp_shr<4>(x1);
  double z = (lane & 4) ? x1 : x0;
  z = z + dpp_shl<2>(z);
  z = z + dpp_shl<1>(z);
  return z;
}

__device__ __forceinline__ double reduce_rows2(double a0, double a1) {
  swap32(a0, a1);
  double p = a0 + a1, q = p;
  swap16(p, q);
  return row16_tree(p + q);
}

__device__ __forceinline__ double block_reduce_256(double v, double *lds4) {
  v = group_reduce<64>(v);
  const int wave = threadIdx.x >> 6;
  if ((threadIdx.x & 63) == 0) lds4[wave] = v;
  __syncthreads();
  return (lds4[0] + lds4[1]) + (lds4[2] + lds4[3]);
}

template <int L, int EPI, bool SPARSE, int BLK = kBlock>
__device__ __forceinline__ void spmv_rows(int64_t block, int64_t nblocks, int64_t nrows,
                                          const int64_t *__restrict__ rp, const int32_t *__restrict__ col,
                                          const double *__restrict__ val, const int32_t *__restrict__ rows,
                                          const double *__restrict__ x, const double *__restrict__ x_halo,
                                          int32_t n_local, double *__restrict__ y, double alpha,
                                          const double *__restrict__ d, double *__restrict__ y2) {
  constexpr int RPB = BLK / L;
  const int lane = threadIdx.x % L;
  const int sub = threadIdx.x / L;
  const int64_t ngroups = (nrows + RPB - 1) / RPB;
  for (int64_t g = block; g < ngroups; g += nblocks) {
    const int64_t r = g * RPB + sub;
    if (r < nrows) {
      const int64_t k0 = rp[r], k1 = rp[r + 1];
      double acc = 0.0;
      for (int64_t k = k0 + lane; k < k1; k += L) {
        const int32_t c = col[k];
        const double xv = (c < n_local) ? x[c] : x_halo[c - n_local];
        acc = fma(val[k], xv, acc);
      }
      acc = group_reduce<L>(acc);
      if (lane == 0) {
        const int64_t ro = SPARSE ? (int64_t)rows[r] : r;
        if (EPI == 0)
          y[ro] = acc;
        else if (EPI == 1)
          y[ro] = fma(alpha, acc, y[ro]);
        else if (EPI == 2)
          y[ro] = d[ro] * acc;
        else {
          y[ro] = acc;
          y2[ro] = d[ro] * acc;
        }
      }
    }
  }
}

template <int L, int EPI, bool SPARSE>
__global__ __launch_bounds__(kBlock) void spmv_kernel(int64_t nrows, const int64_t *__restrict__ rp,
                                                      const int32_t *__restrict__ col,
                                                      const double *__restrict__ val,
                                                      const int32_t *__restrict__ rows,
                                                      const double *__restrict__ x,
                                                      const double *__restrict__ x_halo, int32_t n_local,
                                                      double *__restrict__ y, double alpha,
                                                      const double *__restrict__ d,
                                                      double *__restrict__ y2) {
  spmv_rows<L, EPI, SPARSE>(blockIdx.x, gridDim.x, nrows, rp, col, val, rows, x, x_halo, n_local, y, alpha, d, y2);
}

struct PairC {
  int64_t nrows;
  const int64_t *rp;
  const int32_t *col;
  const double *val, *x_halo, *d;
  double *t;
  int32_t n_local, L;
  uint32_t nA, nC;
};
struct NoPair {};

__device__ __forceinline__ uint32_t pair_nA(const NoPair &) { return gridDim.x; }
__device__ __forceinline__ uint32_t pair_nA(const PairC &c) { return c.nA; }

template <int BLK = kBlock>
__device__ __forceinline__ bool pair_rows(const NoPair &, const double *) { return false; }
template <int BLK = kBlock>
__device__ __forceinline__ bool pair_rows(const PairC &c, const double *__restrict__ x) {
  if (blockIdx.x < c.nA) return false;
  const int64_t block = blockIdx.x - c.nA;
  switch (c.L) {
    case 16: spmv_rows<16, 2, false, BLK>(block, c.nC, c.nrows, c.rp, c.col, c.val, nullptr, x, c.x_halo, c.n_local, c.t, 0.0, c.d, nullptr); break;
    case 32: spmv_rows<32, 2, false, BLK>(block, c.nC, c.nrows, c.rp, c.col, c.val, nullptr, x, c.x_halo, c.n_local, c.t, 0.0, c.d, nullptr); break;
    default: spmv_rows<64, 2, false, BLK>(block, c.nC, c.nrows, c.rp, c.col, c.val, nullptr, x, c.x_halo, c.n_local, c.t, 0.0, c.d, nullptr); break;
  }
  return true;
}
template <bool PAIR>
using PairArg = typename std::conditional<PAIR, PairC, NoPair>::type;

template <int R, int U, int EPI, bool NT, bool PAIR = false>
__global__ __launch_bounds__(kBlock) void spmv_stream_kernel(
    int64_t nrows, const int64_t *__restrict__ rp, const int32_t *__restrict__ col,
    const double *__restrict__ val, const double *__restrict__ x, const double *__restrict__ x_halo,
    int32_t n_local, double *__restrict__ y, double alpha, const double *__restrict__ d,
    double *__restrict__ y2, PairArg<PAIR> pc) {
  if (pair_rows(pc, x)) return;
  const int lane = threadIdx.x & 63;
  const int wave = __builtin_amdgcn_readfirstlane(threadIdx.x >> 6);
  const int64_t nbatches = (nrows + R - 1) / R;
  for (int64_t b = (int64_t)blockIdx.x * 4 + wave; b < nbatches; b += (int64_t)pair_nA(pc) * 4) {
    const int64_t r0 = b * R;
    int64_t kb[R + 1];
#pragma unroll
    for (int i = 0; i <= R; ++i) kb[i] = rp[r0 + i < nrows ? r0 + i : nrows];
    const int64_t k_begin = kb[0];
    const int32_t n_batch = (int32_t)(kb[R] - k_begin);
    int32_t rel[R + 1];
#pragma unroll
    for (int i = 0; i <= R; ++i) rel[i] = (int32_t)(kb[i] - k_begin);
    double acc[R];
#pragma unroll
    for (int i = 0; i < R; ++i) acc[i] = 0.0;
    const int32_t *cb = col + k_begin;
    const double *vb = val + k_begin;
    for (int32_t base = 0; base < n_batch; base += 64 * U) {
      int32_t c[U];
      double v[U], xv[U];
#pragma unroll
      for (int u = 0; u < U; ++u) {
        const int32_t o = base + 64 * u + lane;
        if (o < n_batch) {
          c[u] = NT ? __builtin_nontemporal_load(cb + o) : cb[o];
          v[u] = NT ? __builtin_nontemporal_load(vb + o) : vb[o];
        } else {
          c[u] = -1;
          v[u] = 0.0;
        }
      }
#pragma unroll
      for (int u = 0; u < U; ++u) {
        xv[u] = 0.0;
        if (c[u] >= 0) xv[u] = (c[u] < n_local) ? x[c[u]] : x_halo[c[u] - n_local];
      }
#pragma unroll
      for (int u = 0; u < U; ++u) {
        const int32_t o = base + 64 * u + lane;
        if (c[u] >= 0) {
#pragma unroll
          for (int i = 0; i < R; ++i)
            if (o >= rel[i] && o < rel[i + 1]) acc[i] = fma(v[u], xv[u], acc[i]);
// ... 2173 lines not shown
```

### fictitious_domain_al_preconditioners_amd/solver.py

```python
from __future__ import annotations

import ctypes as C
import os

import numpy as np

from . import _abi

_HERE = os.path.dirname(os.path.abspath(__file__))
LIB_PATH = os.path.join(_HERE, "lib", "libalfd.so")
_lib = None

ABI_SYMBOLS = [
    "alfd_abi_version", "alfd_strerror", "alfd_last_error", "alfd_create", "alfd_destroy",
    "alfd_comm_unique_id", "alfd_comm_init", "alfd_set_partition", "alfd_set_matrix", "alfd_set_diag",
    "alfd_configure", "alfd_default_config", "alfd_setup", "alfd_precond_apply", "alfd_system_apply",
    "alfd_augment_rhs", "alfd_solve", "alfd_upload_rhs", "alfd_solve_resident", "alfd_download_solution",
    "alfd_get_history", "alfd_spmv", "alfd_dot", "alfd_matrix_lanes", "alfd_bench_spmv",
    "alfd_enable_timing", "alfd_get_timing", "alfd_host_halo_plan", "alfd_local_group_create",
    "alfd_local_group_destroy", "alfd_comm_init_local", "alfd_set_aggregates",
    "alfd_set_aggregate_partition", "alfd_get_matrix_info", "alfd_bench_spmv_format",
    "alfd_host_window_plan", "alfd_set_tunable", "alfd_build_aggregates", "alfd_get_aggregates",
    "alfd_host_aggregate_level", "alfd_comm_init_host",
    "alfd_get_device_memory", "alfd_set_row_blocks", "alfd_host_stream_plan",
    "alfd_host_row_blocks_from_points", "alfd_host_stream_plan_short", "alfd_set_prolongator", "alfd_set_controls", "alfd_get_timing_streamed", "alfd_get_setup_seconds",
    "alfd_host_numbering_from_points", "alfd_host_brick_blocks_from_points", "alfd_host_permute_csr",
    "alfd_build_smoothed_aggregation", "alfd_get_prolongator", "alfd_host_smoothed_prolongator",
    "alfd_build_smoothed_aggregation_truncated", "alfd_host_truncate_prolongator",
    "alfd_inner_prec_apply", "alfd_spmv_scaled", "alfd_spmv_pair",
    "alfd_estimate_spectrum", "alfd_get_cg_coefficients", "alfd_host_tridiagonal_extremes",
    "alfd_constraint_residual",
    "alfd_set_prolongator_block", "alfd_build_smoothed_aggregation_block", "alfd_get_prolongator_block",
    "alfd_clear_hierarchy", "alfd_get_inner_iterations", "alfd_get_aggregates_block",
    "alfd_host_strength_graph", "alfd_host_aggregate_graph", "alfd_build_strength_graph", "alfd_get_strength_graph",
    "alfd_upload_rhs_device", "alfd_download_solution_device", "alfd_solve_device", "alfd_precond_apply_device",
    "alfd_system_apply_device", "alfd_augment_rhs_device",
    "alfd_get_matrix_shape", "alfd_get_operator_shape", "alfd_bench_operator", "alfd_host_small_shape",
    "alfd_host_sparse_product", "alfd_sparse_product", "alfd_smoothed_prolongator",
    "alfd_setup_coupling", "alfd_get_setup_counts",
]


class AlfdError(RuntimeError):

    def __init__(self, status, message):
        super().__init__(f"alfd status {status}: {message}")
        self.status = status


class NoConvergence(AlfdError):
    pass


def load_library():
    global _lib
    if _lib is not None:
        return _lib
    if not os.path.exists(LIB_PATH):
        raise ImportError(f"{LIB_PATH} is missing: the HIP extension is required (no CPU fallback). "
                          "Build it with `python -c 'import __graft_entry__ as g; g.build()'`.")
    lib = C.CDLL(LIB_PATH)
    vp, i32, i64, dbl = C.c_void_p, C.c_int32, C.c_int64, C.c_double
    PP = C.POINTER(C.c_void_p)
    sig = {
        "alfd_abi_version": (C.c_int, []),
        "alfd_strerror": (C.c_char_p, [C.c_int]),
        "alfd_last_error": (C.c_char_p, [vp]),
        "alfd_create": (C.c_int, [C.POINTER(vp), C.c_int]),
        "alfd_destroy": (C.c_int, [vp]),
        "alfd_comm_unique_id": (C.c_int, [vp, C.c_size_t]),
        "alfd_comm_init": (C.c_int, [vp, C.c_int, C.c_int, vp, C.c_size_t]),
        "alfd_set_partition": (C.c_int, [vp, C.c_int, PP]),
        "alfd_set_matrix": (C.c_int, [vp, C.c_int, i64, i64, vp, vp, vp]),
        "alfd_set_diag": (C.c_int, [vp, C.c_int, i64, vp]),
        "alfd_configure": (C.c_int, [vp, C.POINTER(_abi.Config)]),
        "alfd_default_config": (None, [C.POINTER(_abi.Config), C.c_int]),
        "alfd_setup": (C.c_int, [vp]),
        "alfd_setup_coupling": (C.c_int, [vp]),
        "alfd_get_setup_counts": (C.c_int, [vp, vp]),
        "alfd_precond_apply": (C.c_int, [vp, PP, PP, C.POINTER(_abi.Result)]),
        "alfd_system_apply": (C.c_int, [vp, PP, PP]),
        "alfd_augment_rhs": (C.c_int, [vp, PP]),
        "alfd_solve": (C.c_int, [vp, PP, PP, C.POINTER(_abi.Result)]),
        "alfd_upload_rhs": (C.c_int, [vp, PP, PP]),
        "alfd_solve_resident": (C.c_int, [vp, C.POINTER(_abi.Result)]),
        "alfd_download_solution": (C.c_int, [vp, PP]),
        "alfd_get_history": (C.c_int, [vp, vp, i32, C.POINTER(i32)]),
        "alfd_spmv": (C.c_int, [vp, C.c_int, vp, vp, C.c_int, dbl]),
        "alfd_spmv_scaled": (C.c_int, [vp, C.c_int, vp, vp, vp, vp]),
        "alfd_spmv_pair": (C.c_int, [vp, C.c_int, C.c_int, vp, vp, vp, vp]),
        "alfd_dot": (C.c_int, [vp, i64, vp, vp, C.POINTER(dbl)]),
        "alfd_inner_prec_apply": (C.c_int, [vp, C.c_int, vp, vp]),
        "alfd_matrix_lanes": (C.c_int, [vp, C.c_int, C.POINTER(i32)]),
        "alfd_bench_spmv": (C.c_int, [vp, C.c_int, i32, C.POINTER(dbl), C.POINTER(dbl)]),
        "alfd_enable_timing": (C.c_int, [vp, C.c_int]),
        "alfd_get_timing": (C.c_int, [vp, vp, vp, vp]),
        "alfd_host_halo_plan": (C.c_int, [i64, vp, vp, C.c_int, C.c_int, vp, vp, i64, C.POINTER(i64), vp]),
        "alfd_local_group_create": (C.c_int, [C.c_int, C.POINTER(vp)]),
        "alfd_local_group_destroy": (C.c_int, [vp]),
        "alfd_comm_init_local": (C.c_int, [vp, vp, C.c_int]),
        "alfd_set_aggregates": (C.c_int, [vp, C.c_int, i64, vp, vp, i64]),
        "alfd_set_aggregate_partition": (C.c_int, [vp, C.c_int, vp]),
        "alfd_set_prolongator": (C.c_int, [vp, C.c_int, i64, i64, vp, vp, vp]),
        "alfd_set_controls": (C.c_int, [vp, vp, vp, vp]),
        "alfd_get_timing_streamed": (C.c_int, [vp, vp]),
        "alfd_get_setup_seconds": (C.c_int, [vp, vp]),
        "alfd_get_matrix_info": (C.c_int, [vp, C.c_int, C.POINTER(_abi.MatrixInfo)]),
        "alfd_bench_spmv_format": (C.c_int, [vp, C.c_int, i32, C.c_int, C.POINTER(dbl), C.POINTER(dbl)]),
        "alfd_get_matrix_shape": (C.c_int, [vp, C.c_int, C.POINTER(_abi.BatchMajorShape)]),
        "alfd_get_operator_shape": (C.c_int, [vp, C.c_int, C.c_int, C.POINTER(_abi.BatchMajorShape)]),
        "alfd_bench_operator": (C.c_int, [vp, C.c_int, C.c_int, i32, i32, i32, C.POINTER(dbl), C.POINTER(_abi.BatchMajorShape)]),
        "alfd_host_small_shape": (C.c_int, [i64, i64, i64, i32, i32, i32, C.POINTER(i32), C.POINTER(i32)]),
        "alfd_host_window_plan": (C.c_int, [i64, vp, vp, vp, i32, i32, C.POINTER(_abi.WindowPlanInfo)]),
        "alfd_set_tunable": (C.c_int, [vp, C.c_char_p, C.c_int]),
        "alfd_build_aggregates": (C.c_int, [vp, i32, dbl, i32, i64, i32, C.POINTER(i32)]),
        "alfd_get_aggregates": (C.c_int, [vp, C.c_int, vp, i64, C.POINTER(i64), C.POINTER(i64)]),
        "alfd_host_aggregate_level": (C.c_int, [i64, vp, vp, vp, i32, dbl, i32, vp, C.POINTER(i64)]),
        "alfd_build_smoothed_aggregation": (C.c_int, [vp, i32, dbl, i32, dbl, i64, i32, C.POINTER(i32), vp]),
        "alfd_build_smoothed_aggregation_truncated": (C.c_int, [vp, i32, dbl, i32, dbl, dbl, i32, i64, i32,
                                                                C.POINTER(i32), vp]),
        "alfd_host_truncate_prolongator": (C.c_int, [i64, i64, vp, vp, vp, vp, i32, dbl, i32, vp, vp, vp, i64,
                                                     C.POINTER(i64)]),
        "alfd_get_prolongator": (C.c_int, [vp, C.c_int, vp, vp, vp, i64, C.POINTER(i64), C.POINTER(i64),
                                           C.POINTER(i64)]),
        "alfd_host_smoothed_prolongator": (C.c_int, [i64, vp, vp, vp, i64, vp, vp, vp, vp, dbl, vp, i64, dbl,
                                                     vp, vp, vp, i64, C.POINTER(i64)]),
        "alfd_host_sparse_product": (C.c_int, [i64, i64, vp, vp, vp, i64, vp, vp, vp, vp, vp, vp, i64, C.POINTER(i64)]),
        "alfd_sparse_product": (C.c_int, [vp, i64, i64, vp, vp, vp, i64, vp, vp, vp, vp, vp, vp, i64, C.POINTER(i64),
                                          C.POINTER(i32)]),
        "alfd_smoothed_prolongator": (C.c_int, [vp, i64, vp, vp, vp, i64, vp, vp, vp, vp, dbl, vp, i64, dbl, i32, dbl, i32,
                                                vp, vp, vp, i64, C.POINTER(i64), C.POINTER(i32)]),
        "alfd_comm_init_host": (C.c_int, [vp, C.c_int, C.c_int, vp, vp, vp]),
        "alfd_get_device_memory": (C.c_int, [vp, C.POINTER(i64), C.POINTER(i64)]),
        "alfd_set_row_blocks": (C.c_int, [vp, C.c_int, i64, vp, vp]),
        "alfd_host_stream_plan": (C.c_int, [i64, vp, vp, vp, C.c_int32, i64, vp, vp, vp]),
        "alfd_host_row_blocks_from_points": (C.c_int, [i64, C.c_int32, vp, C.c_int32, vp, vp, vp]),
        "alfd_host_stream_plan_short": (C.c_int, [i64, vp, vp, vp, C.c_int32, vp]),
        "alfd_host_numbering_from_points": (C.c_int, [i64, C.c_int32, vp, vp]),
        "alfd_host_brick_blocks_from_points": (C.c_int, [i64, C.c_int32, vp, vp, C.c_int32, vp, vp, vp]),
        "alfd_host_permute_csr": (C.c_int, [i64, vp, vp, vp, vp, vp, vp, vp, vp]),
        "alfd_estimate_spectrum": (C.c_int, [vp, C.c_int, C.POINTER(_abi.Control), C.POINTER(_abi.Spectrum)]),
        "alfd_get_cg_coefficients": (C.c_int, [vp, vp, vp, i32, C.POINTER(i32)]),
        "alfd_host_tridiagonal_extremes": (C.c_int, [i32, vp, vp, C.POINTER(dbl), C.POINTER(dbl)]),
        "alfd_constraint_residual": (C.c_int, [vp, PP, vp, C.POINTER(dbl)]),
        "alfd_set_prolongator_block": (C.c_int, [vp, C.c_int, C.c_int, i64, i64, vp, vp, vp]),
        "alfd_build_smoothed_aggregation_block": (C.c_int, [vp, C.c_int, i32, dbl, i32, dbl, dbl, i32, i64, i32,
                                                            C.POINTER(i32), vp]),
        "alfd_get_prolongator_block": (C.c_int, [vp, C.c_int, C.c_int, vp, vp, vp, i64, C.POINTER(i64), C.POINTER(i64),
                                                 C.POINTER(i64)]),
        "alfd_clear_hierarchy": (C.c_int, [vp, C.c_int]),
        "alfd_get_aggregates_block": (C.c_int, [vp, C.c_int, C.c_int, vp, i64, C.POINTER(i64), C.POINTER(i64)]),
        "alfd_get_inner_iterations": (C.c_int, [vp, vp]),
        "alfd_host_strength_graph": (C.c_int, [i64, vp, vp, vp, i32, dbl, vp, vp, vp, vp, vp, i64, C.POINTER(i64)]),
        "alfd_host_aggregate_graph": (C.c_int, [i64, vp, vp, vp, vp, i32, i32, vp, C.POINTER(i64)]),
        "alfd_build_strength_graph": (C.c_int, [vp, i32, dbl, C.POINTER(i64), C.POINTER(i64)]),
        "alfd_get_strength_graph": (C.c_int, [vp, vp, vp, vp, vp, vp, i64, C.POINTER(i32)]),
        "alfd_upload_rhs_device": (C.c_int, [vp, PP, PP, vp]),
        "alfd_download_solution_device": (C.c_int, [vp, PP, vp]),
        "alfd_solve_device": (C.c_int, [vp, PP, PP, C.POINTER(_abi.Result), vp]),
        "alfd_precond_apply_device": (C.c_int, [vp, PP, PP, C.POINTER(_abi.Result), vp]),
        "alfd_system_apply_device": (C.c_int, [vp, PP, PP, vp]),
        "alfd_augment_rhs_device": (C.c_int, [vp, PP, vp]),
    }
    for name, (res, args) in sig.items():
        fn = getattr(lib, name)
        fn.restype = res
        fn.argtypes = args
    _lib = lib
    return lib


def _hip_runtimes():
    try:
        with open("/proc/self/maps") as f:
            return sorted({line.split()[-1] for line in f if "libamdhip64" in line})
    except OSError:
        return []


def _blocks(arrs):
    a = (C.c_void_p * len(arrs))()
    for i, x in enumerate(arrs):
        a[i] = x.ctypes.data
    return a


class Context:

    def __init__(self, device_id=0):
        self._lib = load_library()
        self._h = C.c_void_p()
        rc = self._lib.alfd_create(C.byref(self._h), device_id)
        if rc != _abi.OK:
            self._h = None
            raise AlfdError(rc, "alfd_create failed: " + self._lib.alfd_strerror(rc).decode() +
# ... 325 lines not shown
        x = np.ascontiguousarray(x, np.float64)
        d = np.ascontiguousarray(d, np.float64)
        y = np.ascontiguousarray(y, np.float64).copy()
        t = np.ascontiguousarray(t, np.float64).copy()
        if d.size != t.size:
            raise ValueError("d and t have the row count of slot_c")
        self._ck(self._lib.alfd_spmv_pair(self._h, slot_a, slot_c, x.ctypes.data, d.ctypes.data, y.ctypes.data,
                                          t.ctypes.data))
        return y, t

    def dot(self, x, y):
        x = np.ascontiguousarray(x, np.float64)
        y = np.ascontiguousarray(y, np.float64)
        out = C.c_double()
        self._ck(self._lib.alfd_dot(self._h, x.size, x.ctypes.data, y.ctypes.data, C.byref(out)))
        return out.value

    def inner_prec_apply(self, r, op=_abi.INNER_OP_AUG):
        r = np.ascontiguousarray(r, np.float64)
        bs = self.block_sizes
        if bs is None:
            n = r.size
        else:
            n = {_abi.INNER_OP_AUG: bs[0], _abi.INNER_OP_A22: bs[1]}.get(op, bs[0] + bs[1])
            if r.size != n:
                raise ValueError(f"r has {r.size} entries, the inner operator {n}")
        z = np.zeros(n)
        self._ck(self._lib.alfd_inner_prec_apply(self._h, int(op), r.ctypes.data, z.ctypes.data))
        return z

    def estimate_spectrum(self, op=_abi.SPECTRUM_CCT, control=None):
        out = _abi.Spectrum()
        self._ck(self._lib.alfd_estimate_spectrum(self._h, int(op), None if control is None else C.byref(control),
                                                  C.byref(out)))
        return out

    def cg_coefficients(self):
        cnt = C.c_int32(0)
        self._ck(self._lib.alfd_get_cg_coefficients(self._h, None, None, 0, C.byref(cnt)))
        alpha, beta = np.zeros(cnt.value), np.zeros(max(cnt.value, 1))
        self._ck(self._lib.alfd_get_cg_coefficients(self._h, alpha.ctypes.data, beta.ctypes.data, cnt.value,
                                                    C.byref(cnt)))
        return alpha, beta[:max(cnt.value - 1, 0)].copy()

    def constraint_residual(self, x, g=None):
        x = self._in(x)
        gv = None if g is None else np.ascontiguousarray(g, np.float64)
        if gv is not None and gv.size != self.block_sizes[-1]:
            raise ValueError(f"g has {gv.size} entries, the multiplier block {self.block_sizes[-1]}")
        out = C.c_double()
        self._ck(self._lib.alfd_constraint_residual(self._h, _blocks(x), None if gv is None else gv.ctypes.data,
                                                    C.byref(out)))
        return out.value

    def bench_spmv(self, slot, reps=20):
        ms, nbytes = C.c_double(), C.c_double()
        self._ck(self._lib.alfd_bench_spmv(self._h, slot, reps, C.byref(ms), C.byref(nbytes)))
        return ms.value, nbytes.value

    def bench_spmv_format(self, slot, reps=20, value_index=True):
        ms, nbytes = C.c_double(), C.c_double()
        self._ck(self._lib.alfd_bench_spmv_format(self._h, slot, reps, int(value_index), C.byref(ms),
                                                  C.byref(nbytes)))
        return ms.value, nbytes.value

    def matrix_info(self, slot):
        info, shape = _abi.MatrixInfo(), _abi.BatchMajorShape()
        self._ck(self._lib.alfd_get_matrix_info(self._h, slot, C.byref(info)))
        self._ck(self._lib.alfd_get_matrix_shape(self._h, slot, C.byref(shape)))
        out = {k: getattr(info, k) for k, _ in info._fields_ if k != "reserved"}
        out.update({k: v for k, v in shape.as_dict().items() if k not in out})
        return out

    def operator_info(self, op, level=0):
        shape = _abi.BatchMajorShape()
        self._ck(self._lib.alfd_get_operator_shape(self._h, op, level, C.byref(shape)))
        return shape.as_dict()

    def bench_operator(self, op, level=0, rows=0, waves=0, reps=200):
        us, shape = C.c_double(), _abi.BatchMajorShape()
        self._ck(self._lib.alfd_bench_operator(self._h, op, level, rows, waves, reps, C.byref(us), C.byref(shape)))
        return us.value, shape.as_dict()

    def set_tunable(self, name, value):
        self._ck(self._lib.alfd_set_tunable(self._h, name.encode(), int(value)))

    def sparse_product(self, A, P):
        on = C.c_int32(-1)
        out = _two_call_product(lambda *a: self._lib.alfd_sparse_product(self._h, *a, C.byref(on)), A, P, self._ck)
        return out, bool(on.value)

    def smoothed_prolongator(self, A, agg, n_coarse, omega, Ct=None, w_inv=None, gamma=0.0, block_size=1,
                             drop_tolerance=0.0, max_row_entries=0):
        on = C.c_int32(-1)
        tail = (int(block_size), float(drop_tolerance), int(max_row_entries))
        out = _two_call_prolongator(
            lambda head, *res: self._lib.alfd_smoothed_prolongator(self._h, *head, *tail, *res, C.byref(on)),
            A, agg, n_coarse, omega, Ct, w_inv, gamma, self._ck)
        return out, bool(on.value)

    def set_row_blocks(self, slot, block_ptr, rows):
        if block_ptr is None:
            self._ck(self._lib.alfd_set_row_blocks(self._h, slot, 0, None, None))
            return
        bp = np.ascontiguousarray(block_ptr, np.int64)
        rw = np.ascontiguousarray(rows, np.int32)
        self._ck(self._lib.alfd_set_row_blocks(self._h, slot, bp.size - 1, bp.ctypes.data, rw.ctypes.data))

    def device_memory(self):
        f, t = C.c_int64(0), C.c_int64(0)
        self._ck(self._lib.alfd_get_device_memory(self._h, C.byref(f), C.byref(t)))
        return f.value, t.value

    def enable_timing(self, on=True):
        self._ck(self._lib.alfd_enable_timing(self._h, int(on)))

    def timing(self):
        ms = np.zeros(_abi.T_NCLASSES)
        n = np.zeros(_abi.T_NCLASSES, np.int64)
        b = np.zeros(_abi.T_NCLASSES)
        self._ck(self._lib.alfd_get_timing(self._h, ms.ctypes.data, n.ctypes.data, b.ctypes.data))
        fb = np.zeros(_abi.T_NCLASSES)
        self._ck(self._lib.alfd_get_timing_streamed(self._h, fb.ctypes.data))
        names = ["spmv_A", "spmv_other", "dot", "vec"]
        return {k: dict(ms=float(ms[i]), launches=int(n[i]), bytes=float(b[i]), format_bytes=float(fb[i]))
                for i, k in enumerate(names)}

    def setup_seconds(self):
        s = np.zeros(8)
        self._ck(self._lib.alfd_get_setup_seconds(self._h, s.ctypes.data))
        names = ["upload", "diag_lambda", "ml_fetch", "ml_galerkin", "ml_upload", "ml_lambda", "ml_patch", "ml_coarse"]
        return {k: float(s[i]) for i, k in enumerate(names)}


class LocalGroup:

    def __init__(self, nranks):
        self._lib = load_library()
        self.handle = C.c_void_p()
        rc = self._lib.alfd_local_group_create(nranks, C.byref(self.handle))
        if rc != _abi.OK:
            raise AlfdError(rc, "alfd_local_group_create failed")
        self.nranks = nranks

    def close(self):
        if self.handle:
            self._lib.alfd_local_group_destroy(self.handle)
            self.handle = None


def host_halo_plan(col, col_offsets, rank):
    lib = load_library()
    col = np.ascontiguousarray(col, np.int32)
    offs = np.ascontiguousarray(col_offsets, np.int64)
    nranks = offs.size - 1
    col_local = np.empty_like(col)
    halo = np.empty(max(col.size, 1), np.int32)
    n_halo = C.c_int64()
    recv_off = np.zeros(nranks + 1, np.int64)
    rc = lib.alfd_host_halo_plan(col.size, col.ctypes.data, offs.ctypes.data, nranks, rank,
                                 col_local.ctypes.data, halo.ctypes.data, halo.size, C.byref(n_halo),
                                 recv_off.ctypes.data)
    if rc != _abi.OK:
        raise AlfdError(rc, "alfd_host_halo_plan failed")
    return col_local, halo[:n_halo.value].copy(), recv_off

# ... 446 lines not shown
```

### include/alfd/alfd.h

```cpp
#ifndef ALFD_H
#define ALFD_H

#include <stddef.h>
#include <stdint.h>

#ifdef __cplusplus
extern "C" {
#endif

#define ALFD_ABI_VERSION 12
#define ALFD_MAX_BLOCKS 3

enum alfd_status {
  ALFD_OK = 0,
  ALFD_E_INVALID = 1,
  ALFD_E_HIP = 2,
  ALFD_E_NO_CONVERGENCE_OUTER = 3,
  ALFD_E_NO_CONVERGENCE_INNER = 4,
  ALFD_E_BREAKDOWN = 5,
  ALFD_E_NOT_SETUP = 6,
  ALFD_E_COMM = 7,
  ALFD_E_UNSUPPORTED = 8
};

// ... 190 lines not shown
                        int64_t *nnz, int32_t *on_device);
int alfd_smoothed_prolongator(alfd_ctx_t ctx, int64_t nrows, const int64_t *row_ptr, const int32_t *col, const double *val,
                              int64_t n_mult, const int64_t *ct_row_ptr, const int32_t *ct_col, const double *ct_val,
                              const double *w_inv, double gamma, const int32_t *agg, int64_t n_coarse, double omega,
                              int32_t block_size, double drop_tolerance, int32_t max_row_entries, int64_t *p_row_ptr,
                              int32_t *p_col, double *p_val, int64_t capacity, int64_t *nnz, int32_t *on_device);
int alfd_configure(alfd_ctx_t ctx, const alfd_config *cfg);
int alfd_set_controls(alfd_ctx_t ctx, const alfd_control *outer, const alfd_control *inner, const alfd_control *mp_inner);
void alfd_default_config(alfd_config *cfg, int variant);
int alfd_setup(alfd_ctx_t ctx);
int alfd_setup_coupling(alfd_ctx_t ctx);
enum alfd_setup_count {
  ALFD_SC_PRODUCTS_A = 0,
  ALFD_SC_PRODUCTS_C = 1,
  ALFD_SC_LEVEL_A_UPLOADS = 2,
  ALFD_SC_TRANSFER_UPLOADS = 3,
  ALFD_SC_PATCH_BUILDS = 4,
  ALFD_SC_POWER_ITERATIONS = 5,
  ALFD_SC_NCOUNTS = 6
};
int alfd_get_setup_counts(alfd_ctx_t ctx, int64_t *counts );

int alfd_precond_apply(alfd_ctx_t ctx, const double *const *src_blocks, double *const *dst_blocks,
                       alfd_result *res);
int alfd_system_apply(alfd_ctx_t ctx, const double *const *src_blocks, double *const *dst_blocks);
int alfd_augment_rhs(alfd_ctx_t ctx, double *const *rhs_blocks);
int alfd_solve(alfd_ctx_t ctx, const double *const *rhs_blocks, double *const *x_blocks,
               alfd_result *res);
int alfd_upload_rhs(alfd_ctx_t ctx, const double *const *rhs_blocks, const double *const *x0_blocks);
int alfd_solve_resident(alfd_ctx_t ctx, alfd_result *res);
int alfd_download_solution(alfd_ctx_t ctx, double *const *x_blocks);
int alfd_upload_rhs_device(alfd_ctx_t ctx, const double *const *rhs_blocks, const double *const *x0_blocks,
                           void *stream);
int alfd_download_solution_device(alfd_ctx_t ctx, double *const *x_blocks, void *stream);
int alfd_solve_device(alfd_ctx_t ctx, const double *const *rhs_blocks, double *const *x_blocks, alfd_result *res,
                      void *stream);
int alfd_precond_apply_device(alfd_ctx_t ctx, const double *const *src_blocks, double *const *dst_blocks,
                              alfd_result *res, void *stream);
int alfd_system_apply_device(alfd_ctx_t ctx, const double *const *src_blocks, double *const *dst_blocks, void *stream);
int alfd_augment_rhs_device(alfd_ctx_t ctx, double *const *rhs_blocks, void *stream);
int alfd_get_inner_iterations(alfd_ctx_t ctx, int64_t counts[3]);
int alfd_get_history(alfd_ctx_t ctx, double *out, int32_t capacity, int32_t *count);

int alfd_spmv(alfd_ctx_t ctx, int slot, const double *x, double *y, int mode, double alpha);
int alfd_spmv_scaled(alfd_ctx_t ctx, int slot, const double *x, const double *d, double *y, double *y2);
int alfd_spmv_pair(alfd_ctx_t ctx, int slot_a, int slot_c, const double *x, const double *d, double *y, double *t);
int alfd_dot(alfd_ctx_t ctx, int64_t n, const double *x, const double *y, double *result);
enum alfd_inner_op { ALFD_INNER_OP_AUG = 0, ALFD_INNER_OP_A22 = 1, ALFD_INNER_OP_AUG2 = 2 };
int alfd_inner_prec_apply(alfd_ctx_t ctx, int op, const double *r, double *z);
typedef struct alfd_spectrum {
  int32_t converged;
  int32_t steps;
  double initial_residual, last_residual;
  double lambda_min, lambda_max, condition;
} alfd_spectrum;
enum alfd_spectrum_op { ALFD_SPECTRUM_CCT = 0 };
int alfd_estimate_spectrum(alfd_ctx_t ctx, int op, const alfd_control *ctrl ,
                           alfd_spectrum *out);
int alfd_get_cg_coefficients(alfd_ctx_t ctx, double *alpha, double *beta, int32_t capacity, int32_t *count);
int alfd_host_tridiagonal_extremes(int32_t k, const double *alpha, const double *beta, double *lambda_min, double *lambda_max);
int alfd_constraint_residual(alfd_ctx_t ctx, const double *const *x_blocks, const double *g , double *linf);
int alfd_matrix_lanes(alfd_ctx_t ctx, int slot, int32_t *lanes);
int alfd_bench_spmv(alfd_ctx_t ctx, int slot, int32_t reps, double *ms_per_launch,
                    double *algorithmic_bytes);
typedef struct alfd_matrix_info {
  int32_t lanes, windowed, value_indexed;
  int32_t batch_major;
  int64_t nnz, window_blocks, window_fallback_blocks;
  int64_t value_indexed_blocks, value_indexed_nnz, dictionary_entries, value_wide_nnz;
  double algorithmic_bytes, streamed_bytes;
  int64_t shared_nnz;
  int64_t batch_major_blocks;
  int64_t batch_major_wide;
  int64_t batch_major_interior_blocks;
} alfd_matrix_info;
int alfd_get_matrix_info(alfd_ctx_t ctx, int slot, alfd_matrix_info *out);
typedef struct alfd_batch_major_shape {
  int32_t batch_major, lanes;
  int64_t nrows, nnz, shared_nnz;
  int64_t rows, waves, small;
  int64_t blocks, batches, lds_bytes;
  int64_t compute_units;
} alfd_batch_major_shape;
enum alfd_operator { ALFD_OPERATOR_LEVEL = 0, ALFD_OPERATOR_PATCH_SS = 1, ALFD_OPERATOR_PATCH_S = 2 };
int alfd_get_matrix_shape(alfd_ctx_t ctx, int slot, alfd_batch_major_shape *out);
int alfd_get_operator_shape(alfd_ctx_t ctx, int op, int level, alfd_batch_major_shape *out);
int alfd_bench_operator(alfd_ctx_t ctx, int op, int level, int32_t rows, int32_t waves, int32_t reps,
                        double *us_per_launch, alfd_batch_major_shape *info);
int alfd_host_small_shape(int64_t nrows, int64_t blocks, int64_t batches, int32_t rows, int32_t waves,
                          int32_t compute_units, int32_t *rows_out, int32_t *waves_out);
typedef struct alfd_window_plan_info {
  int32_t windowed, value_indexed, row_block, max_window;
  int64_t blocks, fallback_blocks, segments;
  int64_t value_indexed_blocks, value_indexed_nnz, value_wide_nnz, dictionary_entries;
  int64_t batches, decode_mismatches;
} alfd_window_plan_info;
int alfd_host_window_plan(int64_t nrows, const int64_t *row_ptr, const int32_t *col, const double *val,
                          int32_t lanes, int32_t want_value_index, alfd_window_plan_info *out);
typedef struct alfd_stream_plan_info {
  int32_t ok, max_window, max_rows, max_batches;
  int64_t blocks, batches, segments, dictionary_entries, stream_bytes;
  int64_t decode_mismatches, rows_covered;
  int64_t shared_nnz;
} alfd_stream_plan_info;
int alfd_host_stream_plan(int64_t nrows, const int64_t *row_ptr, const int32_t *col, const double *val,
                          int32_t row_block, int64_t n_blocks, const int64_t *block_ptr, const int32_t *rows,
                          alfd_stream_plan_info *out);
int alfd_host_stream_plan_short(int64_t nrows, const int64_t *row_ptr, const int32_t *col, const double *val,
                                int32_t lanes, alfd_stream_plan_info *out);
int alfd_bench_spmv_format(alfd_ctx_t ctx, int slot, int32_t reps, int use_value_index,
                           double *ms_per_launch, double *streamed_bytes);
int alfd_set_row_blocks(alfd_ctx_t ctx, int slot, int64_t n_blocks, const int64_t *block_ptr, const int32_t *rows);

int alfd_host_row_blocks_from_points(int64_t nrows, int32_t dim, const double *points, int32_t max_rows,
                                     int64_t *n_blocks_out, int64_t *block_ptr_out, int32_t *rows_out);

int alfd_host_numbering_from_points(int64_t nrows, int32_t dim, const double *points, int64_t *new_to_old);
int alfd_host_brick_blocks_from_points(int64_t nrows, int32_t dim, const double *points, const int32_t *brick,
                                       int32_t max_rows, int64_t *n_blocks_out, int64_t *block_ptr_out, int32_t *rows_out);
int alfd_host_permute_csr(int64_t nrows, const int64_t *row_ptr, const int32_t *col, const double *val,
                          const int64_t *row_new_to_old, const int64_t *col_old_to_new, int64_t *out_row_ptr,
                          int32_t *out_col, double *out_val);

int alfd_get_device_memory(alfd_ctx_t ctx, int64_t *free_bytes, int64_t *total_bytes);
int alfd_set_tunable(alfd_ctx_t ctx, const char *name, int value);
enum alfd_timing_class {
  ALFD_T_SPMV_A = 0,
  ALFD_T_SPMV_OTHER = 1,
  ALFD_T_DOT = 2,
  ALFD_T_VEC = 3,
  ALFD_T_NCLASSES = 4
};
int alfd_enable_timing(alfd_ctx_t ctx, int on);
int alfd_get_timing(alfd_ctx_t ctx, double *ms , int64_t *launches ,
                    double *algorithmic_bytes );
int alfd_get_timing_streamed(alfd_ctx_t ctx, double *streamed_bytes );
enum alfd_setup_phase {
  ALFD_SETUP_UPLOAD = 0,
  ALFD_SETUP_DIAG_LAMBDA = 1,
  ALFD_SETUP_ML_FETCH = 2,
  ALFD_SETUP_ML_GALERKIN = 3,
  ALFD_SETUP_ML_UPLOAD = 4,
  ALFD_SETUP_ML_LAMBDA = 5,
  ALFD_SETUP_ML_PATCH = 6,
  ALFD_SETUP_ML_COARSE = 7,
  ALFD_SETUP_NPHASES = 8
};
int alfd_get_setup_seconds(alfd_ctx_t ctx, double *seconds );

#ifdef __cplusplus
}
#endif
#endif
```

Measured before the change: 15.95.

## Add packed dictionary-compressed SpMV form for short-row operators with timed selection

```diff
diff --git a/fictitious_domain_al_preconditioners_amd/_abi.py b/fictitious_domain_al_preconditioners_amd/_abi.py
--- a/fictitious_domain_al_preconditioners_amd/_abi.py
+++ b/fictitious_domain_al_preconditioners_amd/_abi.py
@@ -106,6 +106,21 @@
 
 
 OPERATOR_LEVEL, OPERATOR_PATCH_SS, OPERATOR_PATCH_S = 0, 1, 2
+OPERATOR_PROLONGATION = 3
+
+FORM_CSR, FORM_WINDOW, FORM_BATCH_MAJOR, FORM_PACKED = 0, 1, 2, 3
+
+
+class ShortRowForm(C.Structure):
+    _fields_ = [
+        ("form", C.c_int32), ("lanes", C.c_int32), ("packed_built", C.c_int32), ("dictionary_entries", C.c_int32),
+        ("unroll", C.c_int32), ("reserved", C.c_int32),
+        ("nrows", C.c_int64), ("nnz", C.c_int64), ("packed_device_bytes", C.c_int64),
+        ("form_bytes", C.c_double), ("timed_held_us", C.c_double), ("timed_packed_us", C.c_double),
+    ]
+
+    def as_dict(self):
+        return {k: getattr(self, k) for k, _ in self._fields_ if k != "reserved"}
 
 
 class WindowPlanInfo(C.Structure):
diff --git a/fictitious_domain_al_preconditioners_amd/csrc/alfd.hip b/fictitious_domain_al_preconditioners_amd/csrc/alfd.hip
--- a/fictitious_domain_al_preconditioners_amd/csrc/alfd.hip
+++ b/fictitious_domain_al_preconditioners_amd/csrc/alfd.hip
@@ -43,6 +43,7 @@
   } while (0)
 
 static inline int64_t pad_chunk(int64_t n) { return (n + kChunk - 1) / kChunk * kChunk; }
+constexpr int64_t kShortRowTimedNnz = 20000000;
 
 struct DevCsr {
   bool present = false;
@@ -97,7 +98,19 @@
     int64_t nb_interior = 0;
     double *dict = nullptr;
   } vs;
-  double streamed_bytes(bool use_vi, bool use_vs = false) const {
+  struct Pk {
+    bool built = false, on = false;
+    int32_t ndict = 0, U = 4;
+    uint32_t *ro = nullptr, *ent = nullptr;
+    double *dict = nullptr;
+    int64_t device_bytes = 0;
+    double held_us = 0.0, packed_us = 0.0;
+  } pk;
+  double packed_bytes() const {
+    return (double)nnz * 4.0 + (double)(nrows + 1) * 4.0 + (double)pk.ndict * 8.0 + (double)nrows * 8.0 + (double)ncols * 8.0;
+  }
+  double streamed_bytes(bool use_vi, bool use_vs = false, bool use_pk = false) const {
+    if (pk.on && use_pk) return packed_bytes();
     const double vec = (double)(n_list + 1) * 8.0 + (double)n_list * 8.0 + (double)(sparse ? n_list : ncols) * 8.0;
     if (vs.on && use_vs && use_vi)
       return (double)vs.stream_bytes + 8.0 * vs.tab_u64 * (double)vs.nbatch + 28.0 * (double)vs.nb +
@@ -320,6 +333,8 @@
   int win_short_scale = 2;
   int vs_enable = 1, vs_NW = 4, vs_RB = 96, vs_xcd = 0, vs_share = 1, vs_wide = 1;
   int vs_small = 1;
+  int pk_mode = 1;
+  int pk_U[4] = {2, 2, 4, 4};
   int vs_cus = 0;
   int vs_force_RB = 0, vs_force_NW = 0;
   int vs_lds_base_ok = -1;
@@ -542,6 +557,46 @@
     else ALFD_SPMV(3, false);
   }
 #undef ALFD_SPMV
+}
+
+static inline int packed_grid(int64_t nrows, int L, int U) {
+  const int64_t G = (int64_t)(kBlock / L) * U;
+  return (int)std::max<int64_t>(1, std::min<int64_t>((nrows + G - 1) / G, 256 * 8));
+}
+template <int L, int U>
+static void launch_packed_LU(alfd_ctx *ctx, const DevCsr &m, const double *x, double *y, int epi, double alpha,
+                             const double *d, double *y2) {
+  const int grid = packed_grid(m.nrows, L, U);
+#define ALFD_PK(EPI)                                                                                              \
+  hipLaunchKernelGGL((spmv_packed_kernel<L, EPI, U>), dim3(grid), dim3(kBlock), 0, ctx->stream, m.nrows, m.pk.ro, \
+                     m.pk.ent, m.pk.dict, m.pk.ndict, x, m.halo, m.n_local_cols, y, alpha, d, y2)
+  if (epi == 0) ALFD_PK(0);
+  else if (epi == 1) ALFD_PK(1);
+  else if (epi == 2) ALFD_PK(2);
+  else ALFD_PK(3);
+#undef ALFD_PK
+}
+template <int L>
+static bool launch_packed_L(alfd_ctx *ctx, const DevCsr &m, int U, const double *x, double *y, int epi, double alpha,
+                            const double *d, double *y2) {
+  switch (U) {
+    case 1: launch_packed_LU<L, 1>(ctx, m, x, y, epi, alpha, d, y2); return true;
+    case 2: launch_packed_LU<L, 2>(ctx, m, x, y, epi, alpha, d, y2); return true;
+    case 4: launch_packed_LU<L, 4>(ctx, m, x, y, epi, alpha, d, y2); return true;
+    case 8: launch_packed_LU<L, 8>(ctx, m, x, y, epi, alpha, d, y2); return true;
+  }
+  return false;
+}
+static bool launch_packed(alfd_ctx *ctx, const DevCsr &m, int U, const double *x, double *y, int epi, double alpha,
+                          const double *d, double *y2) {
+  if (!m.pk.built || m.sparse) return false;
+  switch (m.L) {
+    case 4: return launch_packed_L<4>(ctx, m, U, x, y, epi, alpha, d, y2);
+    case 8: return launch_packed_L<8>(ctx, m, U, x, y, epi, alpha, d, y2);
+    case 16: return launch_packed_L<16>(ctx, m, U, x, y, epi, alpha, d, y2);
+    case 32: return launch_packed_L<32>(ctx, m, U, x, y, epi, alpha, d, y2);
+  }
+  return false;
 }
 
 template <int R, int U, bool NT>
@@ -800,12 +855,16 @@
     if (epi == 3) HIPC(hipMemsetAsync(y2, 0, m.nrows * sizeof(double), ctx->stream));
   }
   if (m.n_list == 0) return ALFD_OK;
-  Timer tm(ctx, cls, m.algorithmic_bytes(), m.streamed_bytes(!ctx->vi_off, ctx->vs_enable != 0 && !ctx->vi_off));
+  Timer tm(ctx, cls, m.algorithmic_bytes(), m.streamed_bytes(!ctx->vi_off, ctx->vs_enable != 0 && !ctx->vi_off, ctx->pk_mode != 0));
   return spmv_launch_local(ctx, m, x, y, epi, alpha, d, y2);
 }
 
 static int spmv_launch_local(alfd_ctx *ctx, DevCsr &m, const double *x, double *y, int epi, double alpha, const double *d,
                              double *y2) {
+  if (m.pk.on && ctx->pk_mode && launch_packed(ctx, m, m.pk.U, x, y, epi, alpha, d, y2)) {
+    HIPC(hipGetLastError());
+    return ALFD_OK;
+  }
   if (m.vs.on && ctx->vs_enable && !ctx->vi_off && launch_vs(ctx, m, x, y, epi, alpha, d, y2)) {
     HIPC(hipGetLastError());
     return ALFD_OK;
@@ -833,8 +892,15 @@
   return ALFD_OK;
 }
 
+static void packed_release(DevCsr &m);
 static int pick_short_row_format(alfd_ctx *ctx, DevCsr &m) {
-  if (!m.vs.on || m.vs.L == 64 || m.nnz < 20000000 || ctx->vi_off || !ctx->vs_enable || m.sparse) return ALFD_OK;
+  const bool two = m.vs.on && m.vs.L != 64 && !ctx->vi_off && ctx->vs_enable;
+  if (m.pk.built && ctx->pk_mode == 2) m.pk.on = true;
+  const bool pk = m.pk.built && ctx->pk_mode == 1;
+  if (m.nnz < kShortRowTimedNnz || m.sparse || (!two && !pk)) {
+    if (pk) packed_release(m);
+    return ALFD_OK;
+  }
   double *x = nullptr, *y = nullptr;
   const int64_t nx = std::max<int64_t>(ctx->nranks > 1 && !m.rep ? m.n_local_cols : m.ncols, 1);
   HIPC(hipMalloc((void **)&x, nx * sizeof(double)));
@@ -843,15 +909,19 @@
   hipEvent_t e0, e1;
   HIPC(hipEventCreate(&e0));
   HIPC(hipEventCreate(&e1));
-  float t[2] = {0.f, 0.f};
+  float t[3] = {0.f, 0.f, 0.f};
   bool ok = true;
-  for (int f = 0; f < 2 && ok; ++f) {
+  const bool vs_held = m.vs.on, pk_held = m.pk.on;
+  for (int f = 0; f < 3 && ok; ++f) {
+    if ((f == 0 && !two) || (f == 2 && !pk)) continue;
     for (int it = 0; it < 6 && ok; ++it) {
       if (it == 1) hipEventRecord(e0, ctx->stream);
       m.vs.on = f == 0;
+      m.pk.on = f == 2;
       ok = spmv_launch_local(ctx, m, x, y, 0, 0.0, nullptr, nullptr) == ALFD_OK;
     }
-    m.vs.on = true;
+    m.vs.on = vs_held;
+    m.pk.on = pk_held;
     hipEventRecord(e1, ctx->stream);
     hipEventSynchronize(e1);
     hipEventElapsedTime(&t[f], e0, e1);
@@ -861,11 +931,23 @@
   hipFree(x);
   hipFree(y);
   HIPC(hipGetLastError());
-  if (ok && t[1] < 0.9f * t[0]) {
+  const bool log = ctx->cfg.log_level > 0 || std::getenv("ALFD_LOG_UPLOAD");
+  float held = two ? t[0] : t[1];
+  if (ok && two && t[1] < 0.9f * t[0]) {
     m.vs.on = false;
-    if (ctx->cfg.log_level > 0 || std::getenv("ALFD_LOG_UPLOAD"))
+    held = t[1];
+    if (log)
       std::fprintf(stderr, "[alfd] short-row operator (%lld rows, %lld nnz): without the batch-major form %.3f ms, with it %.3f ms per launch "
                    "-> batch-major form dropped\n", (long long)m.nrows, (long long)m.nnz, t[1] / 5.0, t[0] / 5.0);
+  }
+  if (pk) {
+    m.pk.held_us = 200.0 * held, m.pk.packed_us = 200.0 * t[2];
+    m.pk.on = ok && t[2] < 0.9f * held;
+    if (log)
+      std::fprintf(stderr, "[alfd] short-row operator (%lld rows, %lld nnz, %d lanes): %.3f ms per launch as held, %.3f ms packed (%d values, "
+                   "%d rows in flight per thread) -> %s\n", (long long)m.nrows, (long long)m.nnz, m.L, held / 5.0, t[2] / 5.0, m.pk.ndict,
+                   m.pk.U, m.pk.on ? "packed form" : "packed copy released");
+    if (!m.pk.on) packed_release(m);
   }
   return ALFD_OK;
 }
@@ -3106,6 +3188,116 @@
   return ALFD_OK;
 }
 
+static bool packed_eligible(int64_t nrows, int64_t ncols_with_halo, int64_t nnz, int64_t distinct_values, int lanes, bool sparse) {
+  return nrows >= 0 && lanes >= 4 && lanes <= 32 && !sparse && ncols_with_halo <= ((int64_t)1 << kPackedColBits) &&
+         nnz >= 0 && nnz < ((int64_t)1 << 32) && distinct_values <= kPackedDict;
+}
+
+namespace {
+struct PackedDict {
+  static constexpr int kSlots = 1024;
+  uint64_t key[kSlots];
+  int16_t code[kSlots];
+  std::vector<uint64_t> vals;
+  PackedDict() { std::fill(code, code + kSlots, (int16_t)-1); }
+  int get(uint64_t v) {
+    uint32_t h = (uint32_t)((v * 0x9E3779B97F4A7C15ull) >> 54);
+    while (code[h] >= 0) {
+      if (key[h] == v) return code[h];
+      h = (h + 1) & (kSlots - 1);
+    }
+    if ((int)vals.size() == kPackedDict) return -1;
+    key[h] = v;
+    code[h] = (int16_t)vals.size();
+    vals.push_back(v);
+    return code[h];
+  }
+};
+}
+
+static bool pack_short_rows(int64_t nrows, const int64_t *rp, const int32_t *col, const double *val, uint32_t *ro,
+                            uint32_t *ent, std::vector<double> &dict) {
+  const int64_t nnz = rp[nrows];
+  dict.clear();
+  if (nnz < 0 || nnz >= ((int64_t)1 << 32)) return false;
+  for (int64_t r = 0; r <= nrows; ++r) ro[r] = (uint32_t)rp[r];
+  const int T = nnz < 4000000 ? 1 : (int)std::max(1u, std::min(16u, std::thread::hardware_concurrency()));
+  std::vector<PackedDict> part(T);
+  std::vector<char> bad(T, 0);
+  auto share = [&](int t, int64_t *a, int64_t *b) { *a = nnz * t / T, *b = nnz * (t + 1) / T; };
+  auto run = [&](auto fn) {
+    std::vector<std::thread> th;
+    for (int t = 1; t < T; ++t) th.emplace_back(fn, t);
+    fn(0);
+    for (auto &q : th) q.join();
+  };
+  run([&](int t) {
+    int64_t a, b;
+    share(t, &a, &b);
+    for (int64_t k = a; k < b; ++k) {
+      uint64_t v;
+      std::memcpy(&v, &val[k], 8);
+      if (part[t].get(v) < 0 || col[k] < 0 || (int64_t)col[k] >= ((int64_t)1 << kPackedColBits)) {
+        bad[t] = 1;
+        return;
+      }
+    }
+  });
+  PackedDict all;
+  for (int t = 0; t < T; ++t) {
+    if (bad[t]) return false;
+    for (uint64_t v : part[t].vals)
+      if (all.get(v) < 0) return false;
+  }
+  run([&](int t) {
+    PackedDict mine = all;
+    int64_t a, b;
+    share(t, &a, &b);
+    for (int64_t k = a; k < b; ++k) {
+      uint64_t v;
+      std::memcpy(&v, &val[k], 8);
+      ent[k] = ((uint32_t)mine.get(v) << kPackedColBits) | (uint32_t)col[k];
+    }
+  });
+  dict.resize(all.vals.size());
+  if (!dict.empty()) std::memcpy(dict.data(), all.vals.data(), 8 * dict.size());
+  return true;
+}
+
+static void packed_release(DevCsr &m) {
+  for (void *q : {(void *)m.pk.ro, (void *)m.pk.ent, (void *)m.pk.dict}) {
+    auto it = std::find(m.owned.begin(), m.owned.end(), q);
+    if (q && it != m.owned.end()) {
+      hipFree(q);
+      m.owned.erase(it);
+    }
+  }
+  const double held = m.pk.held_us, packed = m.pk.packed_us;
+  m.pk = DevCsr::Pk();
+  m.pk.held_us = held, m.pk.packed_us = packed;
+}
+
+static int build_packed(alfd_ctx *ctx, DevCsr &m, const int64_t *rp, const int32_t *col, const double *val, bool any_size) {
+  if (!ctx->pk_mode || m.nnz == 0 || !(any_size || m.nnz >= kShortRowTimedNnz)) return ALFD_OK;
+  if (!packed_eligible(m.nrows, (int64_t)m.n_local_cols + m.n_halo, m.nnz, 0, m.L, m.sparse)) return ALFD_OK;
+  std::vector<uint32_t> ro((size_t)m.nrows + 1), ent((size_t)m.nnz);
+  std::vector<double> dict;
+  if (!pack_short_rows(m.nrows, rp, col, val, ro.data(), ent.data(), dict)) return ALFD_OK;
+  RC(csr_alloc(ctx, m, &m.pk.ro, m.nrows + 1));
+  RC(csr_alloc(ctx, m, &m.pk.ent, m.nnz));
+  RC(csr_alloc(ctx, m, &m.pk.dict, (int64_t)kPackedDict));
+  HIPC(hipMemcpyAsync(m.pk.ro, ro.data(), ro.size() * sizeof(uint32_t), hipMemcpyHostToDevice, ctx->stream));
+  HIPC(hipMemcpyAsync(m.pk.ent, ent.data(), ent.size() * sizeof(uint32_t), hipMemcpyHostToDevice, ctx->stream));
+  HIPC(hipMemsetAsync(m.pk.dict, 0, kPackedDict * sizeof(double), ctx->stream));
+  HIPC(hipMemcpyAsync(m.pk.dict, dict.data(), dict.size() * sizeof(double), hipMemcpyHostToDevice, ctx->stream));
+  HIPC(hipStreamSynchronize(ctx->stream));
+  m.pk.ndict = (int32_t)dict.size();
+  m.pk.U = ctx->pk_U[m.L == 4 ? 0 : m.L == 8 ? 1 : m.L == 16 ? 2 : 3];
+  m.pk.device_bytes = 4 * (m.nrows + 1) + 4 * m.nnz + 8 * (int64_t)kPackedDict;
+  m.pk.built = true;
+  return ALFD_OK;
+}
+
 static int upload_matrix(alfd_ctx *ctx, int slot, int64_t nrows, int64_t ncols, const int64_t *rp,
                          const int32_t *col, const double *val) {
   DevCsr &m = ctx->mat[slot];
@@ -3261,6 +3453,7 @@
     if (copy_job.rc != hipSuccess) return ctx->err = hipGetErrorString(copy_job.rc), ALFD_E_HIP;
   }
   m.present = true;
+  RC(build_packed(ctx, m, rp, col_up, val, ctx->pk_mode == 2));
   RC(pick_short_row_format(ctx, m));
   return ALFD_OK;
 }
@@ -6624,6 +6817,11 @@
   if (const char *e = std::getenv("ALFD_SPMV_BATCH_MAJOR")) ctx->vs_enable = std::atoi(e);
   if (const char *e = std::getenv("ALFD_SPMV_BATCH_MAJOR_ROWS")) ctx->vs_RB = std::max(4, std::min(kVsMaxRows, std::atoi(e)));
   if (const char *e = std::getenv("ALFD_SPMV_SMALL_SHAPES")) ctx->vs_small = std::atoi(e) != 0;
+  if (const char *e = std::getenv("ALFD_SPMV_PACKED")) ctx->pk_mode = std::max(0, std::min(2, std::atoi(e)));
+  if (const char *e = std::getenv("ALFD_SPMV_PACKED_U")) {
+    const int u = std::atoi(e);
+    if (u == 1 || u == 2 || u == 4 || u == 8) std::fill(ctx->pk_U, ctx->pk_U + 4, u);
+  }
   {
     hipDeviceProp_t prop;
     if (hipGetDeviceProperties(&prop, device_id) == hipSuccess) ctx->vs_cus = prop.multiProcessorCount;
@@ -8241,6 +8439,10 @@
   } else if (op == ALFD_OPERATOR_PATCH_SS || op == ALFD_OPERATOR_PATCH_S) {
     if (!ctx->patch.on) return nullptr;
     m = op == ALFD_OPERATOR_PATCH_SS ? &ctx->patch.Ass : &ctx->patch.As;
+  } else if (op == ALFD_OPERATOR_PROLONGATION) {
+    std::vector<MlLevel> &ml = ctx->hier[0].ml;
+    if (level < 1 || level >= (int)ml.size()) return nullptr;
+    m = ml[level].rep.P.present ? &ml[level].rep.P : &ml[level].loc.P;
   }
   return m && m->present ? m : nullptr;
 }
@@ -8314,6 +8516,122 @@
   if (!ok) return ctx->err = "alfd_bench_operator: launch or timing failed", ALFD_E_HIP;
   if (us_per_launch) *us_per_launch = 1000.0 * (double)ms / reps;
   if (info) shape_of(ctx, *m, info);
+  return ALFD_OK;
+}
+
+static void form_of(const alfd_ctx *ctx, const DevCsr &m, alfd_short_row_form *out) {
+  std::memset(out, 0, sizeof(*out));
+  const bool pk = m.pk.on && ctx->pk_mode != 0, vs = m.vs.on && ctx->vs_enable && !ctx->vi_off;
+  out->form = pk ? ALFD_FORM_PACKED : vs ? ALFD_FORM_BATCH_MAJOR : m.win ? ALFD_FORM_WINDOW : ALFD_FORM_CSR;
+  out->lanes = m.L;
+  out->packed_built = m.pk.built ? 1 : 0;
+  out->dictionary_entries = m.pk.ndict;
+  out->unroll = m.pk.built ? m.pk.U : 0;
+  out->nrows = m.nrows;
+  out->nnz = m.nnz;
+  out->packed_device_bytes = m.pk.device_bytes;
+  out->form_bytes = m.streamed_bytes(!ctx->vi_off, ctx->vs_enable != 0 && !ctx->vi_off, ctx->pk_mode != 0);
+  out->timed_held_us = m.pk.held_us;
+  out->timed_packed_us = m.pk.packed_us;
+}
+
+int alfd_get_matrix_form(alfd_ctx_t ctx, int slot, alfd_short_row_form *out) {
+  CHECK_CTX();
+  if (slot < 0 || slot >= ALFD_NSLOTS || !ctx->mat[slot].present || !out) return ALFD_E_INVALID;
+  form_of(ctx, ctx->mat[slot], out);
+  return ALFD_OK;
+}
+
+int alfd_get_operator_form(alfd_ctx_t ctx, int op, int level, alfd_short_row_form *out) {
+  CHECK_CTX();
+  CHECK_SETUP();
+  const DevCsr *m = own_operator(ctx, op, level);
+  if (!m || !out) return ALFD_E_INVALID;
+  form_of(ctx, *m, out);
+  return ALFD_OK;
+}
+
+int alfd_bench_short_rows(alfd_ctx_t ctx, int op, int level, int slot, int32_t form, int32_t unroll, int32_t reps,
+                          double *us_per_launch, double *form_bytes) {
+  CHECK_CTX();
+  if (ctx->nranks > 1) return ALFD_E_UNSUPPORTED;
+  DevCsr *m = nullptr;
+  if (op >= 0) {
+    CHECK_SETUP();
+    m = own_operator(ctx, op, level);
+  } else if (slot >= 0 && slot < ALFD_NSLOTS && ctx->mat[slot].present) {
+    m = &ctx->mat[slot];
+  }
+  const bool packed = form == ALFD_FORM_PACKED;
+  if (!m || reps < 1 || (packed && unroll != 0 && unroll != 1 && unroll != 2 && unroll != 4 && unroll != 8)) return ALFD_E_INVALID;
+  if (m->sparse || m->nrows == 0) return ctx->err = "alfd_bench_short_rows: no rows, or a row list", ALFD_E_UNSUPPORTED;
+  struct Guard {
+    alfd_ctx *ctx;
+    DevCsr &m;
+    const DevCsr::Pk pk;
+    const int mode;
+    bool built_here = false;
+    ~Guard() {
+      if (built_here) packed_release(m);
+      m.pk = pk;
+      ctx->pk_mode = mode;
+    }
+  } guard{ctx, *m, m->pk, ctx->pk_mode};
+  if (packed && !m->pk.built) {
+    HostCsr h;
+    RC(download_csr(ctx, *m, h));
+    ctx->pk_mode = 2;
+    guard.built_here = true;
+    RC(build_packed(ctx, *m, h.rp.data(), h.col.data(), h.val.data(), true));
+    if (!m->pk.built) return ctx->err = "alfd_bench_short_rows: the operator cannot take the packed form", ALFD_E_UNSUPPORTED;
+  }
+  ctx->pk_mode = packed ? 2 : 0;
+  m->pk.on = packed;
+  if (packed && unroll) m->pk.U = unroll;
+  double *dx = nullptr, *dy = nullptr;
+  HIPC(hipMalloc((void **)&dx, std::max<int64_t>(m->ncols, 1) * sizeof(double)));
+  if (hipMalloc((void **)&dy, m->nrows * sizeof(double)) != hipSuccess) {
+    hipFree(dx);
+    return ctx->err = "alfd_bench_short_rows: out of device memory", ALFD_E_HIP;
+  }
+  hipLaunchKernelGGL(hash_vector_kernel, dim3((unsigned)std::max<int64_t>(1, (m->ncols + 255) / 256)), dim3(256), 0, ctx->stream,
+                     m->ncols, (int64_t)0, dx);
+  hipMemsetAsync(dy, 0, m->nrows * sizeof(double), ctx->stream);
+  hipEvent_t a = nullptr, b = nullptr;
+  float ms = 0;
+  bool ok = hipEventCreate(&a) == hipSuccess && hipEventCreate(&b) == hipSuccess;
+  ok = ok && spmv_launch_local(ctx, *m, dx, dy, 1, 1.0, nullptr, nullptr) == ALFD_OK;
+  ok = ok && hipEventRecord(a, ctx->stream) == hipSuccess;
+  for (int i = 0; ok && i < reps; ++i) ok = spmv_launch_local(ctx, *m, dx, dy, 1, 1.0, nullptr, nullptr) == ALFD_OK;
+  ok = ok && hipEventRecord(b, ctx->stream) == hipSuccess && hipEventSynchronize(b) == hipSuccess &&
+       hipEventElapsedTime(&ms, a, b) == hipSuccess;
+  hipStreamSynchronize(ctx->stream);
+  if (a) hipEventDestroy(a);
+  if (b) hipEventDestroy(b);
+  hipFree(dx);
+  hipFree(dy);
+  if (form_bytes) *form_bytes = m->streamed_bytes(!ctx->vi_off, ctx->vs_enable != 0 && !ctx->vi_off, packed);
+  HIPC(hipGetLastError());
+  if (!ok) return ctx->err = "alfd_bench_short_rows: launch or timing failed", ALFD_E_HIP;
+  if (us_per_launch) *us_per_launch = 1000.0 * (double)ms / reps;
+  return ALFD_OK;
+}
+
+int alfd_host_packed_eligible(int64_t nrows, int64_t ncols_with_halo, int64_t nnz, int64_t distinct_values, int32_t lanes,
+                              int32_t sparse) {
+  return packed_eligible(nrows, ncols_with_halo, nnz, distinct_values, lanes, sparse != 0) ? 1 : 0;
+}
+
+int alfd_host_pack_short_rows(int64_t nrows, const int64_t *rp, const int32_t *col, const double *val, void *row_offsets,
+                              void *entries, double *dictionary, int32_t *dictionary_entries) {
+  if (nrows < 0 || !rp || !row_offsets || !dictionary || !dictionary_entries) return ALFD_E_INVALID;
+  if (rp[nrows] > 0 && (!col || !val || !entries)) return ALFD_E_INVALID;
+  std::vector<double> dict;
+  if (!pack_short_rows(nrows, rp, col, val, static_cast<uint32_t *>(row_offsets), static_cast<uint32_t *>(entries), dict))
+    return ALFD_E_UNSUPPORTED;
+  std::fill(dictionary, dictionary + kPackedDict, 0.0);
+  if (!dict.empty()) std::memcpy(dictionary, dict.data(), 8 * dict.size());
+  *dictionary_entries = (int32_t)dict.size();
   return ALFD_OK;
 }
 
@@ -8732,6 +9050,16 @@
     ctx->vs_small = value != 0;
     return ALFD_OK;
   }
+  if (std::strcmp(name, "short_row_packed") == 0) {
+    if (value < 0 || value > 2) return ctx->err = "short_row_packed: 0, 1 or 2", ALFD_E_INVALID;
+    ctx->pk_mode = value;
+    return ALFD_OK;
+  }
+  if (std::strcmp(name, "short_row_packed_unroll") == 0) {
+    if (value != 1 && value != 2 && value != 4 && value != 8) return ctx->err = "short_row_packed_unroll: 1, 2, 4 or 8", ALFD_E_INVALID;
+    std::fill(ctx->pk_U, ctx->pk_U + 4, value);
+    return ALFD_OK;
+  }
   if (std::strcmp(name, "batch_major_rows") == 0) {
     if (value < 4 || value > kVsMaxRows) return ctx->err = "batch_major_rows: 4..250", ALFD_E_INVALID;
     ctx->vs_RB = value;
diff --git a/fictitious_domain_al_preconditioners_amd/csrc/kernels.hpp b/fictitious_domain_al_preconditioners_amd/csrc/kernels.hpp
--- a/fictitious_domain_al_preconditioners_amd/csrc/kernels.hpp
+++ b/fictitious_domain_al_preconditioners_amd/csrc/kernels.hpp
@@ -199,6 +199,89 @@
                                                       const double *__restrict__ d,
                                                       double *__restrict__ y2) {
   spmv_rows<L, EPI, SPARSE>(blockIdx.x, gridDim.x, nrows, rp, col, val, rows, x, x_halo, n_local, y, alpha, d, y2);
+}
+
+constexpr int kPackedColBits = 24;
+constexpr uint32_t kPackedColMask = (1u << kPackedColBits) - 1u;
+constexpr int kPackedDict = 256;
+
+template <int L, int EPI, int U>
+__global__ __launch_bounds__(kBlock) void spmv_packed_kernel(int64_t nrows, const uint32_t *__restrict__ ro,
+                                                             const uint32_t *__restrict__ ent,
+                                                             const double *__restrict__ dictv, int32_t ndict,
+                                                             const double *__restrict__ x,
+                                                             const double *__restrict__ x_halo, int32_t n_local,
+                                                             double *__restrict__ y, double alpha,
+                                                             const double *__restrict__ d, double *__restrict__ y2) {
+  constexpr int RPB = kBlock / L;
+  constexpr int64_t G = (int64_t)RPB * U;
+  constexpr int C = L <= 8 ? 2 : 1;
+  __shared__ double dict[kPackedDict];
+  dict[threadIdx.x] = (int)threadIdx.x < ndict ? dictv[threadIdx.x] : 0.0;
+  __syncthreads();
+  const int lane = threadIdx.x % L;
+  const int sub = threadIdx.x / L;
+  const int64_t ngroups = (nrows + G - 1) / G;
+  for (int64_t g = blockIdx.x; g < ngroups; g += gridDim.x) {
+    int64_t r[U];
+    uint32_t k0[U], k1[U], e[U][C];
+    double acc[U], xv[U][C], yo[U];
+#pragma unroll
+    for (int u = 0; u < U; ++u) {
+      r[u] = g * G + (int64_t)u * RPB + sub;
+      const bool in = r[u] < nrows;
+      k0[u] = in ? ro[r[u]] : 0u;
+      k1[u] = in ? ro[r[u] + 1] : 0u;
+      if (EPI == 1) yo[u] = (in && lane == 0) ? y[r[u]] : 0.0;
+    }
+#pragma unroll
+    for (int u = 0; u < U; ++u)
+#pragma unroll
+      for (int c = 0; c < C; ++c) {
+        const uint64_t k = (uint64_t)k0[u] + (uint64_t)(lane + c * L);
+        e[u][c] = k < (uint64_t)k1[u] ? ent[k] : 0xffffffffu;
+      }
+#pragma unroll
+    for (int u = 0; u < U; ++u)
+#pragma unroll
+      for (int c = 0; c < C; ++c) {
+        const bool has = (uint64_t)k0[u] + (uint64_t)(lane + c * L) < (uint64_t)k1[u];
+        const int32_t cc = (int32_t)(e[u][c] & kPackedColMask);
+        xv[u][c] = !has ? 0.0 : (cc < n_local) ? x[cc] : x_halo[cc - n_local];
+      }
+#pragma unroll
+    for (int u = 0; u < U; ++u) {
+      acc[u] = 0.0;
+#pragma unroll
+      for (int c = 0; c < C; ++c) {
+        const bool has = (uint64_t)k0[u] + (uint64_t)(lane + c * L) < (uint64_t)k1[u];
+        if (has) acc[u] = fma(dict[e[u][c] >> kPackedColBits], xv[u][c], acc[u]);
+      }
+      for (uint64_t k = (uint64_t)k0[u] + (uint64_t)(lane + C * L); k < (uint64_t)k1[u]; k += L) {
+        const uint32_t ek = ent[k];
+        const int32_t cc = (int32_t)(ek & kPackedColMask);
+        const double xk = (cc < n_local) ? x[cc] : x_halo[cc - n_local];
+        acc[u] = fma(dict[ek >> kPackedColBits], xk, acc[u]);
+      }
+    }
+#pragma unroll
+    for (int u = 0; u < U; ++u) {
+      const double s = group_reduce<L>(acc[u]);
+      if (lane == 0 && r[u] < nrows) {
+        const int64_t ro_ = r[u];
+        if (EPI == 0)
+          y[ro_] = s;
+        else if (EPI == 1)
+          y[ro_] = fma(alpha, s, yo[u]);
+        else if (EPI == 2)
+          y[ro_] = d[ro_] * s;
+        else {
+          y[ro_] = s;
+          y2[ro_] = d[ro_] * s;
+        }
+      }
+    }
+  }
 }
 
 struct PairC {
diff --git a/fictitious_domain_al_preconditioners_amd/solver.py b/fictitious_domain_al_preconditioners_amd/solver.py
--- a/fictitious_domain_al_preconditioners_amd/solver.py
+++ b/fictitious_domain_al_preconditioners_amd/solver.py
@@ -38,6 +38,8 @@
     "alfd_get_matrix_shape", "alfd_get_operator_shape", "alfd_bench_operator", "alfd_host_small_shape",
     "alfd_host_sparse_product", "alfd_sparse_product", "alfd_smoothed_prolongator",
     "alfd_setup_coupling", "alfd_get_setup_counts",
+    "alfd_get_matrix_form", "alfd_get_operator_form", "alfd_bench_short_rows", "alfd_host_packed_eligible",
+    "alfd_host_pack_short_rows",
 ]
 
 
@@ -111,6 +113,11 @@
         "alfd_get_operator_shape": (C.c_int, [vp, C.c_int, C.c_int, C.POINTER(_abi.BatchMajorShape)]),
         "alfd_bench_operator": (C.c_int, [vp, C.c_int, C.c_int, i32, i32, i32, C.POINTER(dbl), C.POINTER(_abi.BatchMajorShape)]),
         "alfd_host_small_shape": (C.c_int, [i64, i64, i64, i32, i32, i32, C.POINTER(i32), C.POINTER(i32)]),
+        "alfd_get_matrix_form": (C.c_int, [vp, C.c_int, C.POINTER(_abi.ShortRowForm)]),
+        "alfd_get_operator_form": (C.c_int, [vp, C.c_int, C.c_int, C.POINTER(_abi.ShortRowForm)]),
+        "alfd_bench_short_rows": (C.c_int, [vp, C.c_int, C.c_int, C.c_int, i32, i32, i32, C.POINTER(dbl), C.POINTER(dbl)]),
+        "alfd_host_packed_eligible": (C.c_int, [i64, i64, i64, i64, i32, i32]),
+        "alfd_host_pack_short_rows": (C.c_int, [i64, vp, vp, vp, vp, vp, vp, C.POINTER(i32)]),
         "alfd_host_window_plan": (C.c_int, [i64, vp, vp, vp, i32, i32, C.POINTER(_abi.WindowPlanInfo)]),
         "alfd_set_tunable": (C.c_int, [vp, C.c_char_p, C.c_int]),
         "alfd_build_aggregates": (C.c_int, [vp, i32, dbl, i32, i64, i32, C.POINTER(i32)]),
@@ -602,6 +609,21 @@
         self._ck(self._lib.alfd_bench_operator(self._h, op, level, rows, waves, reps, C.byref(us), C.byref(shape)))
         return us.value, shape.as_dict()
 
+    def matrix_form(self, slot):
+        out = _abi.ShortRowForm()
+        self._ck(self._lib.alfd_get_matrix_form(self._h, slot, C.byref(out)))
+        return out.as_dict()
+
+    def operator_form(self, op, level=0):
+        out = _abi.ShortRowForm()
+        self._ck(self._lib.alfd_get_operator_form(self._h, op, level, C.byref(out)))
+        return out.as_dict()
+
+    def bench_short_rows(self, op=-1, level=0, slot=-1, form=_abi.FORM_CSR, unroll=0, reps=200):
+        us, nbytes = C.c_double(), C.c_double()
+        self._ck(self._lib.alfd_bench_short_rows(self._h, op, level, slot, form, unroll, reps, C.byref(us), C.byref(nbytes)))
+        return us.value, nbytes.value
+
     def set_tunable(self, name, value):
         self._ck(self._lib.alfd_set_tunable(self._h, name.encode(), int(value)))
 
diff --git a/include/alfd/alfd.h b/include/alfd/alfd.h
--- a/include/alfd/alfd.h
+++ b/include/alfd/alfd.h
@@ -296,13 +296,35 @@
   int64_t blocks, batches, lds_bytes;
   int64_t compute_units;
 } alfd_batch_major_shape;
-enum alfd_operator { ALFD_OPERATOR_LEVEL = 0, ALFD_OPERATOR_PATCH_SS = 1, ALFD_OPERATOR_PATCH_S = 2 };
+enum alfd_operator { ALFD_OPERATOR_LEVEL = 0, ALFD_OPERATOR_PATCH_SS = 1, ALFD_OPERATOR_PATCH_S = 2,
+                     ALFD_OPERATOR_PROLONGATION = 3  };
 int alfd_get_matrix_shape(alfd_ctx_t ctx, int slot, alfd_batch_major_shape *out);
 int alfd_get_operator_shape(alfd_ctx_t ctx, int op, int level, alfd_batch_major_shape *out);
 int alfd_bench_operator(alfd_ctx_t ctx, int op, int level, int32_t rows, int32_t waves, int32_t reps,
                         double *us_per_launch, alfd_batch_major_shape *info);
 int alfd_host_small_shape(int64_t nrows, int64_t blocks, int64_t batches, int32_t rows, int32_t waves,
                           int32_t compute_units, int32_t *rows_out, int32_t *waves_out);
+enum alfd_short_row_form_kind { ALFD_FORM_CSR = 0, ALFD_FORM_WINDOW = 1, ALFD_FORM_BATCH_MAJOR = 2, ALFD_FORM_PACKED = 3 };
+typedef struct alfd_short_row_form {
+  int32_t form;
+  int32_t lanes;
+  int32_t packed_built;
+  int32_t dictionary_entries;
+  int32_t unroll;
+  int32_t reserved;
+  int64_t nrows, nnz;
+  int64_t packed_device_bytes;
+  double form_bytes;
+  double timed_held_us, timed_packed_us;
+} alfd_short_row_form;
+int alfd_get_matrix_form(alfd_ctx_t ctx, int slot, alfd_short_row_form *out);
+int alfd_get_operator_form(alfd_ctx_t ctx, int op, int level, alfd_short_row_form *out);
+int alfd_bench_short_rows(alfd_ctx_t ctx, int op, int level, int slot, int32_t form, int32_t unroll, int32_t reps,
+                          double *us_per_launch, double *form_bytes);
+int alfd_host_packed_eligible(int64_t nrows, int64_t ncols_with_halo, int64_t nnz, int64_t distinct_values,
+                              int32_t lanes, int32_t sparse);
+int alfd_host_pack_short_rows(int64_t nrows, const int64_t *rp, const int32_t *col, const double *val,
+                              void *row_offsets, void *entries, double *dictionary, int32_t *dictionary_entries);
 typedef struct alfd_window_plan_info {
   int32_t windowed, value_indexed, row_block, max_window;
   int64_t blocks, fallback_blocks, segments;
diff --git a/profiles/packed_short_rows/families.py b/profiles/packed_short_rows/families.py
--- /dev/null
+++ b/profiles/packed_short_rows/families.py
@@ -0,0 +1,32 @@
+import collections
+import csv
+import re
+import sys
+
+src, dst = sys.argv[1], sys.argv[2]
+solves = float(sys.argv[3]) if len(sys.argv) > 3 else 2.0
+levels = int(sys.argv[4]) if len(sys.argv) > 4 else 3
+pat = re.compile(r"(spmv_kernel<4, 1, false>|spmv_window_group_kernel<[^>]*>|spmv_packed_kernel<[^>]*>)")
+rows = []
+with open(src) as f:
+    for r in csv.DictReader(f):
+        m = pat.search(r["Kernel_Name"])
+        if m:
+            rows.append((int(r["Start_Timestamp"]), m.group(1), int(r["Grid_Size_X"]) // max(int(r["Workgroup_Size_X"]), 1),
+                         int(r["End_Timestamp"]) - int(r["Start_Timestamp"])))
+rows.sort()
+acc = collections.defaultdict(list)
+seen = collections.Counter()
+for _, name, wg, ns in rows:
+    cls = ""
+    if name == "spmv_kernel<4, 1, false>":
+        cls = f"cycle position {seen[name] % levels}"
+        seen[name] += 1
+    acc[(name, wg, cls)].append(ns)
+with open(dst, "w") as f:
+    w = csv.writer(f)
+    w.writerow(["kernel", "workgroups", "class", "calls_per_solve", "ms_per_solve", "min_us", "avg_us", "max_us"])
+    for (name, wg, cls), t in sorted(acc.items()):
+        w.writerow([name, wg, cls, f"{len(t) / solves:.1f}", f"{sum(t) / solves * 1e-6:.3f}", f"{min(t) * 1e-3:.2f}",
+                    f"{sum(t) / len(t) * 1e-3:.2f}", f"{max(t) * 1e-3:.2f}"])
+print(open(dst).read())
diff --git a/profiles/packed_short_rows/sweep.py b/profiles/packed_short_rows/sweep.py
--- /dev/null
+++ b/profiles/packed_short_rows/sweep.py
@@ -0,0 +1,65 @@
+import argparse, json, os, sys, time
+
+ROOT = os.path.dirname(os.path.dirname(os.path.dirname(os.path.abspath(__file__))))
+sys.path.insert(0, ROOT)
+ap = argparse.ArgumentParser()
+ap.add_argument("--n-cells", type=int, default=74)
+ap.add_argument("--reps", type=int, default=200)
+ap.add_argument("--repeats", type=int, default=3)
+ap.add_argument("--out", default=None)
+args = ap.parse_args()
+
+import numpy as np
+from fictitious_domain_al_preconditioners_amd import _abi, problems, solver
+
+HERE = os.path.dirname(os.path.abspath(__file__))
+out_path = args.out or os.path.join(HERE, f"sweep_n{args.n_cells}.jsonl")
+out_file = open(out_path, "w")
+
+
+def emit(**fields):
+    line = json.dumps(fields, sort_keys=True)
+    print(line, flush=True)
+    out_file.write(line + "\n")
+    out_file.flush()
+
+
+n = args.n_cells
+refine = max(0, int(round(np.log2(n / 64.0))) + 4)
+t0 = time.time()
+pb = problems.stokes3d_sphere(n_cells=n, immersed_refine=refine)
+cfg = _abi.bench_multilevel_settings(_abi.default_config(_abi.AL_STOKES), geometric=True)
+cfg.inner.max_steps = 100
+levels = problems.tensor_prolongators(pb.params, min_coarse=_abi.BENCH_MIN_COARSE)
+ctx = solver.Context(0)
+ctx.set_tunable("short_row_packed", 2)
+solver.upload_problem(ctx, pb, cfg, levels, problems.brick_row_blocks(pb.params, (16, 4, 1)))
+emit(kind="system", n_cells=n, setup_wall_s=round(time.time() - t0, 1), library_phases_s=ctx.setup_seconds())
+
+OPS = [("P_0", dict(op=_abi.OPERATOR_PROLONGATION, level=1)), ("P_1", dict(op=_abi.OPERATOR_PROLONGATION, level=2)),
+       ("Bt", dict(op=-1, slot=_abi.BT))]
+NAMES = {_abi.FORM_CSR: "csr", _abi.FORM_WINDOW: "window group", _abi.FORM_BATCH_MAJOR: "batch-major", _abi.FORM_PACKED: "packed"}
+
+for name, which in OPS:
+    try:
+        held = ctx.operator_form(which["op"], which["level"]) if which["op"] >= 0 else ctx.matrix_form(which["slot"])
+    except solver.AlfdError as e:
+        emit(kind="skipped", operator=name, why=str(e))
+        continue
+    ctx.set_tunable("short_row_packed", 0)
+    under = ctx.operator_form(which["op"], which["level"]) if which["op"] >= 0 else ctx.matrix_form(which["slot"])
+    ctx.set_tunable("short_row_packed", 2)
+    emit(kind="operator", operator=name, nrows=held["nrows"], nnz=held["nnz"], lanes=held["lanes"],
+         dictionary_entries=held["dictionary_entries"], packed_built=held["packed_built"],
+         packed_device_bytes=held["packed_device_bytes"], form_without_packed=NAMES[under["form"]])
+    for k in range(args.repeats):
+        for form, unroll in [(_abi.FORM_CSR, 0)] + [(_abi.FORM_PACKED, u) for u in (1, 2, 4, 8)]:
+            try:
+                us, nbytes = ctx.bench_short_rows(form=form, unroll=unroll, reps=args.reps, **which)
+            except solver.AlfdError as e:
+                emit(kind="time", operator=name, form=NAMES[form], unroll=unroll, repeat=k, error=str(e))
+                continue
+            emit(kind="time", operator=name, form="packed" if form == _abi.FORM_PACKED else NAMES[under["form"]], unroll=unroll,
+                 repeat=k, us_per_launch=round(us, 2), form_bytes=nbytes, gb_per_s=round(nbytes / us * 1e-3, 1))
+ctx.close()
+out_file.close()
```

After: 16.08, median of 6. No clear change (+0.8%).
